# hvak/visual-underwater-slam

Hardware: AMD Instinct MI355X
Metric: ORB detect+match frames/sec (higher is better)
Workload: dtype u8

## Files before the change

### visual-underwater-slam_amd/_lib.py

```python
import ctypes
import os
from ctypes import c_int, c_void_p, c_char_p, c_double

_HERE = os.path.dirname(os.path.abspath(__file__))
LIB_PATH = os.environ.get("VUS_HIP_LIB") or os.path.join(_HERE, "csrc", "libvus_hip.so")

_P = c_void_p

SIGNATURES = {
    "vus_fast_score": [_P, c_int, c_int, c_int, c_int, c_int, _P, _P],
    "vus_blur7": [_P, c_int, c_int, c_int, c_int, _P, _P],
    "vus_fast_detect": [_P, c_int, c_int, c_int, c_int, c_int, c_int, _P, _P, c_int, _P, _P],
    "vus_fast_threshold_estimate": [_P, c_int, c_int, c_int, c_int, c_int, c_int, c_int, c_int, _P, _P, _P],
    "vus_fast_detect_adaptive": [_P, c_int, c_int, c_int, c_int, _P, c_int, _P, _P, c_int, _P, _P],
    "vus_fast_detect_retry": [_P, c_int, c_int, c_int, c_int, c_int, _P, c_int, c_int, _P, c_int, _P, _P, _P, _P],
    "vus_select_topk": [_P, _P, c_int, c_int, c_int, _P, _P, _P],
    "vus_orient_rbrief": [_P, _P, c_int, c_int, c_int, c_int, _P, _P, c_int, _P, _P, _P],
    "vus_orient_order": [_P, _P, c_int, c_int, c_int, c_int, _P, _P],
    "vus_orient_rbrief_ordered": [_P, _P, c_int, c_int, c_int, c_int, _P, _P, c_int, _P, _P, _P, _P],
    "vus_hamming_match": [_P, _P, _P, c_int, c_int, c_int, _P, _P, c_int, c_int, c_int, c_int, c_int, _P, _P, _P],
    "vus_triangulate": [_P, c_int, _P, _P, _P, _P],
    "vus_select_grid": [_P, _P, c_int, c_int, c_int, c_int, c_int, c_int, c_int, c_int, _P, _P, _P],
    "vus_cross_check": [_P, _P, c_int, c_int, _P, _P],
    "vus_resize_bilinear": [_P, c_int, c_int, c_int, c_int, _P, c_int, c_int, c_int, _P],
    "vus_pyramid_append": [_P, _P, _P, _P, c_int, c_int, c_int, c_int, c_int, c_int, c_int, c_int, _P, _P, _P, _P, _P, _P,
                           _P],
    "vus_track_ids": [_P, _P, _P, _P, c_int, c_int, c_int, c_int, _P, _P, _P, _P],
    "vus_stereo_initial_residuals": [_P, _P, _P, _P, _P, _P, c_int, _P, _P],
    "vus_emit_stereo_factors": [_P, _P, _P, _P, c_int, c_int, c_int, ctypes.c_longlong, _P, _P, _P, _P, _P, _P, _P, _P],
    "vus_ba_linearize": [_P, _P, _P, _P, _P, _P, _P, _P, _P, _P, _P],
    "vus_ba_schur": [_P, _P, c_double, _P, _P, _P, _P, _P, _P, _P, _P, c_int, _P, _P, _P],
    "vus_ba_tiles_count": [_P, _P, _P],
    "vus_ba_tiles_fill": [_P, c_int, _P, c_int, _P, _P, _P, _P, ctypes.c_longlong, _P],
    "vus_ba_add_diag": [_P, c_int, c_int, c_double, _P],
    "vus_ba_band_solve": [_P, c_int, c_int, _P, _P, _P, _P],
    "vus_ba_backsub": [_P, _P, _P, _P, _P, _P, _P],
    "vus_ba_eval_step": [_P, _P, _P, _P, _P, _P, _P, _P, _P, _P],
    "vus_ba_error": [_P, _P, _P, _P, _P, _P],
    "vus_ba_band_solve_multi": [_P, c_int, c_int, _P, c_int, _P, _P],
    "vus_ba_band_solve_split": [_P, c_int, c_int, _P, _P, _P, _P, _P],
    "vus_ba_band_solve_multi_split": [_P, c_int, c_int, _P, c_int, _P, _P, _P],
    "vus_ba_linearize_robust": [_P, _P, _P, _P, _P, _P, _P, _P, _P, _P, _P, _P],
    "vus_ba_eval_step_robust": [_P, _P, _P, _P, _P, _P, _P, _P, _P, _P, _P],
    "vus_ba_error_robust": [_P, _P, _P, _P, _P, _P, _P],
    "vus_ba_stereo_weights": [_P, _P, _P, _P, _P, _P],
    "vus_imu_preintegrate": [_P, _P, c_int, _P, _P, _P, _P],
    "vus_keys_to_indices": [_P, c_int, _P, _P, _P, _P, ctypes.c_longlong, _P],
    "vus_lookup_keys": [_P, c_int, _P, c_int, _P, _P, _P],
    "vus_ba_pack_observations": [_P, _P, _P, c_int, c_int, c_int, _P, _P, _P, _P, _P, _P, _P, _P, _P, _P, _P, ctypes.c_longlong, _P],
    "vus_exclusive_scan_i32": [_P, c_int, _P, _P, _P],
    "vus_nav_linearize": [_P, c_int, _P, _P, _P, _P, _P, _P, _P, _P, _P, _P, _P],
    "vus_nav_assemble": [c_int, c_int, c_double, _P, _P, _P, _P, _P, _P, _P],
    "vus_nav_border_solve": [c_int, _P, _P, _P, _P, c_double, _P, _P, _P],
    "vus_nav_eval_step": [_P, c_int, _P, _P, _P, _P, _P, _P, _P, _P, _P, _P, _P],
    "vus_nav_error": [_P, c_int, _P, _P, _P, _P, _P, _P],
    "vus_navb_linearize": [_P, c_int, _P, _P, _P, _P, _P, _P, _P, _P],
    "vus_navb_assemble": [c_int, c_int, c_double, _P, _P, _P, _P, _P],
    "vus_navb_eval_step": [_P, c_int, _P, _P, _P, _P, _P, _P, _P, _P, _P, _P],
    "vus_navb_error": [_P, c_int, _P, _P, _P, _P, _P, _P],
    "vus_ba_band_selinv": [_P, c_int, c_int, _P, _P, ctypes.c_longlong, _P],
    "vus_ba_point_check": [_P, c_int, _P, _P],
    "vus_ba_point_covariance": [_P, _P, _P, _P, _P, c_int, _P, _P],
    "vus_nav_border_covariance": [c_int, c_int, _P, _P, _P, _P, _P, _P, _P, _P],
    "vus_between_check": [_P, c_int, _P],
    "vus_between_linearize": [_P, _P, _P, _P, _P, _P],
    "vus_between_assemble": [_P, _P, c_int, _P, _P, _P],
    "vus_between_eval_step": [_P, _P, _P, _P, _P, _P, _P],
    "vus_between_error": [_P, _P, _P, _P, _P],
    "vus_ba_set_tuning": [c_int, c_int],
}

TUNE_BAND_MODE, TUNE_CB_MAX_WG, TUNE_LAST_BAND_MODE, TUNE_WIN_FAULT = 0, 1, 2, 3
STATUS_WAIT_EXPIRED, STATUS_WINDOW_EXPIRED = -1, -3


class VusError(RuntimeError):
    """A libvus_hip.so entry point returned a negative code (gtsam raises RuntimeError likewise)."""


_lib = None


def load():
    global _lib
    if _lib is not None:
        return _lib
    import torch
    if not os.path.exists(LIB_PATH):
        raise ImportError(
            f"{LIB_PATH} is missing: build it with `python -c 'import __graft_entry__ as g; g.build()'` "
            "or `make -C visual-underwater-slam_amd/csrc`. There is no CPU fallback.")
    lib = ctypes.CDLL(LIB_PATH)
    lib.vus_abi_version.restype = c_int
    lib.vus_last_error.restype = c_char_p
    lib.vus_build_target.restype = c_char_p
    for name, argtypes in SIGNATURES.items():
        fn = getattr(lib, name)
        fn.argtypes = argtypes
        fn.restype = c_int
    lib.vus_ba_work_doubles.argtypes = [_P]
    lib.vus_ba_work_doubles.restype = ctypes.c_longlong
    lib.vus_ba_band_solve_work_doubles.argtypes = [c_int, c_int, c_int]
    lib.vus_ba_band_solve_work_doubles.restype = ctypes.c_longlong
    lib.vus_pack_work_bytes.argtypes = [c_int]
    lib.vus_pack_work_bytes.restype = ctypes.c_longlong
    lib.vus_ba_tiles_work_bytes.argtypes = [c_int]
    lib.vus_ba_tiles_work_bytes.restype = ctypes.c_longlong
    lib.vus_ba_get_tuning.argtypes = [c_int]
    lib.vus_ba_get_tuning.restype = c_int
    lib.vus_nav_work_doubles.argtypes = [_P]
    lib.vus_nav_work_doubles.restype = ctypes.c_longlong
    lib.vus_navb_work_doubles.argtypes = [_P]
    lib.vus_navb_work_doubles.restype = ctypes.c_longlong
    lib.vus_between_work_doubles.argtypes = [_P]
    lib.vus_between_work_doubles.restype = ctypes.c_longlong
    lib.vus_ba_band_selinv_work_doubles.argtypes = [c_int, c_int]
    lib.vus_ba_band_selinv_work_doubles.restype = ctypes.c_longlong
    _lib = lib
    return lib


def call(name, *args):
    lib = load()
    rc = getattr(lib, name)(*args)
    if rc != 0:
        raise VusError(f"{name} failed ({rc}): {_explain_missing_code_object(lib.vus_last_error().decode())}")


def ptr(t):
    return None if t is None else t.data_ptr()


def current_stream_ptr():
    import torch
    return torch.cuda.current_stream().cuda_stream


def target_mismatch(built: str, device_arch: str):
    b, d = built.split(":"), device_arch.split(":")
    if b[0] != d[0]:
        return (f"libvus_hip.so was built for {built} but the device is {device_arch}: this library targets MI355X "
                f"(gfx950) only")
    for feat in b[1:]:
        if feat not in d[1:]:
            return (f"libvus_hip.so was built for target ID {built} but the device runs {device_arch}: no code object "
                    f"matches (every launch would fail with 'no kernel image is available'). Rebuild with "
                    f"`make -C visual-underwater-slam_amd/csrc clean all OFFLOAD=--offload-arch={b[0]}`")
    return None


def _explain_missing_code_object(text: str) -> str:
    if "no kernel image" not in text and "invalid device function" not in text:
        return text
    try:
        import torch
        arch = getattr(torch.cuda.get_device_properties(torch.cuda.current_device()), "gcnArchName", "")
        why = target_mismatch(load().vus_build_target().decode(), arch) if arch else None
    except Exception:
        why = None
    return f"{text} -- {why}" if why else text


def check_target():
    import torch
    arch = getattr(torch.cuda.get_device_properties(torch.cuda.current_device()), "gcnArchName", "")
    why = target_mismatch(load().vus_build_target().decode(), arch) if arch else None
    if why:
        raise RuntimeError(why)


def require_gpu():
    import torch
    if not torch.cuda.is_available():
        raise RuntimeError("visual_underwater_slam_amd needs an MI355X (HIP device); no GPU is visible "
                           "and there is deliberately no CPU fallback.")
```

### visual-underwater-slam_amd/csrc/frontend.hip

```cpp
#include "vus_common.h"
#define VUS_TABLE_QUAL __device__ constexpr
#include "../../include/vus_orb_tables.h"

namespace {

#ifndef VUS_TW
#define VUS_TW 128
#endif
#ifndef VUS_TH
#define VUS_TH 24
#endif
constexpr int TW = VUS_TW;
constexpr int TH = VUS_TH;
#ifndef VUS_AB_TILE
static_assert(TW == VUS_FAST_TILE_W && TH == VUS_FAST_TILE_H, "the sampling pattern of vus_fast_threshold_estimate is part of the ABI");
#endif
#ifndef VUS_FAST_WPE
#define VUS_FAST_WPE 1
#endif
#ifndef VUS_NT
#define VUS_NT 256
#endif
constexpr int NTHREADS = VUS_NT;
constexpr int IMG_ROWS = TH + 8;
constexpr int IMG_DW = (TW + 16) / 4;
constexpr int SC_ROWS = TH + 2;
constexpr int SC_DW = (TW + 8) / 4;
constexpr int H_ROWS = TH + 6;
constexpr int H_DW = TW / 2;
constexpr int STRIPS = TW / 4;

__device__ __forceinline__ int clampi(int v, int lo, int hi) { return v < lo ? lo : (v > hi ? hi : v); }
__device__ __forceinline__ int min3i(int a, int b, int c) { return min(min(a, b), c); }
__device__ __forceinline__ int max3i(int a, int b, int c) { return max(max(a, b), c); }
__device__ __forceinline__ int byte_of(uint32_t w, int i) { return (int)((w >> (8 * i)) & 0xFFu); }

template <int E>
__device__ __forceinline__ int fast_score_strip(const uint32_t (&r)[7][3]) {
  constexpr int DX[16] = {0, 1, 2, 3, 3, 3, 2, 1, 0, -1, -2, -3, -3, -3, -2, -1};
  constexpr int DY[16] = {-3, -3, -2, -1, 0, 1, 2, 3, 3, 3, 2, 1, 0, -1, -2, -3};
  const int p = byte_of(r[3][1], E);
  int d[16];
#pragma unroll
  for (int k = 0; k < 16; ++k) {
    const int pos = 4 + E + DX[k];
    d[k] = byte_of(r[3 + DY[k]][pos >> 2], pos & 3) - p;
  }
  int mn3[16], mx3[16];
#pragma unroll
  for (int k = 0; k < 16; ++k) {
    mn3[k] = min3i(d[k], d[(k + 1) & 15], d[(k + 2) & 15]);
    mx3[k] = max3i(d[k], d[(k + 1) & 15], d[(k + 2) & 15]);
  }
  int best_bright = -(1 << 20), best_dark = 1 << 20;
#pragma unroll
  for (int k = 0; k < 16; ++k) {
    best_bright = max(best_bright, min3i(mn3[k], mn3[(k + 3) & 15], mn3[(k + 6) & 15]));
    best_dark = min(best_dark, max3i(mx3[k], mx3[(k + 3) & 15], mx3[(k + 6) & 15]));
  }
  return max(best_bright, -best_dark) - 1;
}

__device__ __forceinline__ int fast_score_bytes(const uint8_t* c, int rb) {
  constexpr int DX[16] = {0, 1, 2, 3, 3, 3, 2, 1, 0, -1, -2, -3, -3, -3, -2, -1};
  constexpr int DY[16] = {-3, -3, -2, -1, 0, 1, 2, 3, 3, 3, 2, 1, 0, -1, -2, -3};
  const int p = c[0];
  int d[16];
#pragma unroll
  for (int k = 0; k < 16; ++k) d[k] = (int)c[DY[k] * rb + DX[k]] - p;
  int mn3[16], mx3[16];
#pragma unroll
  for (int k = 0; k < 16; ++k) {
    mn3[k] = min3i(d[k], d[(k + 1) & 15], d[(k + 2) & 15]);
    mx3[k] = max3i(d[k], d[(k + 1) & 15], d[(k + 2) & 15]);
  }
  int best_bright = -(1 << 20), best_dark = 1 << 20;
#pragma unroll
  for (int k = 0; k < 16; ++k) {
    best_bright = max(best_bright, min3i(mn3[k], mn3[(k + 3) & 15], mn3[(k + 6) & 15]));
    best_dark = min(best_dark, max3i(mx3[k], mx3[(k + 3) & 15], mx3[(k + 6) & 15]));
  }
  return max(best_bright, -best_dark) - 1;
}

typedef short short2_t __attribute__((ext_vector_type(2)));
__device__ __forceinline__ int fast_score_pk(const uint32_t (&r)[7][3]) {
  constexpr int DX[16] = {0, 1, 2, 3, 3, 3, 2, 1, 0, -1, -2, -3, -3, -3, -2, -1};
  constexpr int DY[16] = {-3, -3, -2, -1, 0, 1, 2, 3, 3, 3, 2, 1, 0, -1, -2, -3};
  const int p = byte_of(r[3][1], 0);
  uint32_t nr[7][2];
#pragma unroll
  for (int k = 0; k < 7; ++k) {
    nr[k][0] = ~r[k][0];
    nr[k][1] = ~r[k][1];
  }
  short2_t v[16];
#pragma unroll
  for (int k = 0; k < 16; ++k) {
    const int pos = 4 + DX[k], row = 3 + DY[k], dw = pos >> 2, by = pos & 3;
    const uint32_t sel = (uint32_t)by | (0x0cu << 8) | ((uint32_t)(4 + by) << 16) | (0x0cu << 24);
    v[k] = __builtin_bit_cast(short2_t, __builtin_amdgcn_perm(nr[row][dw], r[row][dw], sel));
  }
  short2_t w2[16], w4[16], w8[16];
#pragma unroll
  for (int k = 0; k < 16; ++k) w2[k] = __builtin_elementwise_min(v[k], v[(k + 1) & 15]);
#pragma unroll
  for (int k = 0; k < 16; ++k) w4[k] = __builtin_elementwise_min(w2[k], w2[(k + 2) & 15]);
#pragma unroll
  for (int k = 0; k < 16; ++k) w8[k] = __builtin_elementwise_min(w4[k], w4[(k + 4) & 15]);
  short2_t best = __builtin_elementwise_min(w8[0], v[8]);
#pragma unroll
  for (int k = 1; k < 16; ++k) best = __builtin_elementwise_max(best, __builtin_elementwise_min(w8[k], v[(k + 8) & 15]));
  return max((int)best.x - p, (int)best.y - (255 - p)) - 1;
}

#ifndef VUS_FAST_PK
#define VUS_FAST_PK 0
#endif

template <int E>
__device__ __forceinline__ bool nms_keep(const uint32_t (&c)[3][3]) {
  const int s = byte_of(c[1][1], E);
  int m = 0;
#pragma unroll
  for (int dy = 0; dy < 3; ++dy)
#pragma unroll
    for (int dx = -1; dx <= 1; ++dx) {
      if (dy == 1 && dx == 0) continue;
      const int pos = 4 + E + dx;
      m = max(m, byte_of(c[dy][pos >> 2], pos & 3));
    }
  return s > m;
}

#ifndef VUS_FAST_STRIP
#define VUS_FAST_STRIP 1
#endif
#ifndef VUS_BLUR_MFMA
#define VUS_BLUR_MFMA 1
#endif
#ifndef VUS_FAST_LATE_BLUR
#define VUS_FAST_LATE_BLUR 1
#endif
constexpr int VUS_CAND_REGIONS = 8;
#ifndef VUS_FAST_SCORE_BYTES
#define VUS_FAST_SCORE_BYTES 1
#endif
#ifndef VUS_FAST_MM_BYTES
#define VUS_FAST_MM_BYTES 1
#endif
#ifndef VUS_FAST_DIAG
#define VUS_FAST_DIAG 1
#endif
struct BlurMfmaTable {
  uint64_t h[64];
  uint64_t v[2][64];
};
constexpr BlurMfmaTable make_blur_mfma_table() {
  constexpr int BW[7] = {18, 33, 49, 56, 49, 33, 18};
  BlurMfmaTable t{};
  for (int l = 0; l < 64; ++l) {
    const int g = l >> 4, m = l & 15;
    for (int sl = 0; sl < 8; ++sl) {
      const int d = 8 * g + sl - m - 5;
      if (d >= 0 && d <= 6) t.h[l] |= (uint64_t)BW[d] << (8 * sl);
      const int hrow = sl < 4 ? 4 * g + sl : 16 + 4 * g + (sl - 4);
      for (int nb = 0; nb < 2; ++nb) {
        const int dv = hrow - (16 * nb + m + 1);
        if (dv >= 0 && dv <= 6) t.v[nb][l] |= (uint64_t)BW[dv] << (8 * sl);
      }
    }
  }
  return t;
}
__device__ __attribute__((aligned(16))) const BlurMfmaTable g_blur_mfma_table = make_blur_mfma_table();
typedef int v4i32_t __attribute__((ext_vector_type(4)));

__device__ __forceinline__ void blur_tile_mfma(const uint32_t* s_img, uint8_t* __restrict__ blur_out, int n, int H, int W,
                                               int x0, int y0, int tid, int j_first, int j_step) {
  static_assert(IMG_ROWS == 32 && TW % 16 == 0 && (IMG_DW * 4) % 8 == 0, "blur_tile_mfma: K = the 32 staged rows");
  const int l = tid & 63, g = l >> 4, m = l & 15;
  const long bh = (long)g_blur_mfma_table.h[l];
  const long bv[2] = {(long)g_blur_mfma_table.v[0][l], (long)g_blur_mfma_table.v[1][l]};
  const uint8_t* img8 = reinterpret_cast<const uint8_t*>(s_img);
  constexpr unsigned long long SIGN = 0x8080808080808080ull;
#ifndef VUS_BLUR_UNROLL
#define VUS_BLUR_UNROLL 1
#endif
#pragma unroll VUS_BLUR_UNROLL
  for (int j = j_first; j < TW / 16; j += j_step) {
    v4i32_t ch[2];
#pragma unroll
    for (int mb = 0; mb < 2; ++mb) {
      const unsigned long long a =
          *reinterpret_cast<const unsigned long long*>(img8 + (16 * mb + m) * (IMG_DW * 4) + 16 * j + 8 * g) ^ SIGN;
      const v4i32_t c0 = {32768, 32768, 32768, 32768};
      ch[mb] = __builtin_amdgcn_mfma_i32_16x16x32_i8((long)a, bh, c0, 0, 0, 0);
    }
    uint32_t lo[2], hi[2];
#pragma unroll
    for (int mb = 0; mb < 2; ++mb) {
      const uint32_t t0 = __builtin_amdgcn_perm((uint32_t)ch[mb][1], (uint32_t)ch[mb][0], 0x05010400u);
      const uint32_t t1 = __builtin_amdgcn_perm((uint32_t)ch[mb][3], (uint32_t)ch[mb][2], 0x05010400u);
      lo[mb] = __builtin_amdgcn_perm(t1, t0, 0x05040100u);
      hi[mb] = __builtin_amdgcn_perm(t1, t0, 0x07060302u);
    }
    const long a_lo = (long)((((unsigned long long)lo[1] << 32) | lo[0]) ^ SIGN);
    const long a_hi = (long)((((unsigned long long)hi[1] << 32) | hi[0]) ^ SIGN);
#pragma unroll
    for (int nb = 0; nb < 2; ++nb) {
      const v4i32_t ci = {32768, 32768, 32768, 32768};
      const v4i32_t cl = {65536, 65536, 65536, 65536};
      const v4i32_t chi = __builtin_amdgcn_mfma_i32_16x16x32_i8(a_hi, bv[nb], ci, 0, 0, 0);
      const v4i32_t clo = __builtin_amdgcn_mfma_i32_16x16x32_i8(a_lo, bv[nb], cl, 0, 0, 0);
      uint32_t q[4];
#pragma unroll
      for (int r = 0; r < 4; ++r) q[r] = ((uint32_t)chi[r] << 8) + (uint32_t)clo[r];
      const uint32_t v = __builtin_amdgcn_perm(q[1], q[0], 0x0c0c0602u) | __builtin_amdgcn_perm(q[3], q[2], 0x06020c0cu);
      const int ly = 16 * nb + m, gy = y0 + ly, gx = x0 + 16 * j + 4 * g;
#ifdef VUS_BLUR_EXP_NOSTORE
      if (v != 0x12345678u) continue;
#endif
      if (ly < TH && gy < H) {
        uint8_t* o = blur_out + ((size_t)n * H + gy) * W + gx;
        if (gx + 3 < W) {
          __builtin_memcpy(o, &v, 4);
        } else {
#pragma unroll
          for (int e = 0; e < 4; ++e)
            if (gx + e < W) o[e] = (uint8_t)(v >> (8 * e));
        }
      }
    }
  }
}

#ifdef VUS_FAST_DEBUG_COUNT
__device__ unsigned long long g_fast_dbg[4];
extern "C" int vus_debug_fast_counters(unsigned long long* out, int reset) {
  if (hipMemcpyFromSymbol(out, HIP_SYMBOL(g_fast_dbg), sizeof(g_fast_dbg)) != hipSuccess) return -1;
  if (reset) { unsigned long long z[4] = {0, 0, 0, 0}; if (hipMemcpyToSymbol(HIP_SYMBOL(g_fast_dbg), z, sizeof(z)) != hipSuccess) return -1; }
  return 0;
}
#endif
template <bool WRITE_SCORE, bool DETECT, bool BLUR, bool HIST = false, bool REGIONS = false>
__device__ __forceinline__ void fast_tile_body(
    const uint8_t* __restrict__ img, int H, int W, int pitch, int thr, int border,
    uint8_t* __restrict__ score_out, uint8_t* __restrict__ blur_out,
    uint32_t* __restrict__ cand_keys, int cand_cap, int* __restrict__ cand_count, int* __restrict__ hist,
    int n, int tile, int tiles_x) {
  __shared__ __attribute__((aligned(8))) uint32_t s_img[IMG_ROWS * IMG_DW];
  __shared__ uint32_t s_score[(WRITE_SCORE || DETECT) ? SC_ROWS * SC_DW : 1];
  constexpr bool STRIP = VUS_FAST_STRIP && (WRITE_SCORE || DETECT);
  constexpr bool MFMA_BLUR = VUS_BLUR_MFMA && BLUR && IMG_ROWS == 32;
  constexpr int AUX_DW = STRIP ? (IMG_ROWS * IMG_DW + SC_ROWS * SC_DW + 1) / 2 : 2;
  __shared__ uint32_t s_h[(BLUR && !MFMA_BLUR && H_ROWS * H_DW > AUX_DW) ? H_ROWS * H_DW : AUX_DW];
  __shared__ uint16_t s_work[(WRITE_SCORE || DETECT) ? SC_ROWS * SC_DW * 4 : 2];
#if VUS_FAST_STRIP
  uint16_t* const s_mm = reinterpret_cast<uint16_t*>(s_h);
  uint16_t* const s_strip = s_mm + IMG_ROWS * IMG_DW;
  __shared__ int s_nstrip;
#endif
  __shared__ int s_cnt, s_base, s_nwork;
  constexpr bool LATE_BLUR = MFMA_BLUR && DETECT && !HIST && STRIP && VUS_FAST_LATE_BLUR;
  static_assert(IMG_ROWS * IMG_DW >= TW * TH / 4, "candidate list must fit in the image tile");
  static_assert(!LATE_BLUR || AUX_DW >= TW * TH / 4, "candidate list must fit in the strip tables' buffer");
  uint32_t* const s_keys = LATE_BLUR ? s_h : s_img;

  const int tid = threadIdx.x;
  const int x0 = (tile % tiles_x) * TW, y0 = (tile / tiles_x) * TH;
  const uint8_t* im = img + (size_t)n * H * pitch;

  {
    constexpr int RPP = NTHREADS / IMG_DW;
    const int col = tid % IMG_DW, r0 = tid / IMG_DW;
    const int gx = x0 - 8 + 4 * col;
    const bool fast = gx >= 0 && gx + 3 < W;
    const bool inside = x0 >= 8 && x0 + TW + 8 <= W && y0 >= 4 && y0 + TH + 4 <= H;
    if (r0 < RPP) {
      constexpr int NP = (IMG_ROWS + RPP - 1) / RPP;
      constexpr int LASTP = IMG_ROWS - (NP - 1) * RPP;
      uint32_t v[NP];
      if (inside) {
        const uint32_t off0 = (uint32_t)((y0 - 4 + r0) * pitch + gx);
        const uint32_t step = (uint32_t)(RPP * pitch);
#pragma unroll
        for (int k = 0; k < NP - 1; ++k) __builtin_memcpy(&v[k], im + (off0 + (uint32_t)k * step), 4);
        v[NP - 1] = 0u;
        if (r0 < LASTP) __builtin_memcpy(&v[NP - 1], im + (off0 + (uint32_t)(NP - 1) * step), 4);
      } else {
        const uint8_t* rp[NP];
#pragma unroll
        for (int k = 0; k < NP; ++k) rp[k] = im + (size_t)clampi(y0 - 4 + min(r0 + RPP * k, IMG_ROWS - 1), 0, H - 1) * pitch;
        if (fast) {
#pragma unroll
          for (int k = 0; k < NP; ++k) __builtin_memcpy(&v[k], rp[k] + gx, 4);
        } else {
          const int c0 = clampi(gx, 0, W - 1), c1 = clampi(gx + 1, 0, W - 1), c2 = clampi(gx + 2, 0, W - 1),
                    c3 = clampi(gx + 3, 0, W - 1);
          uint8_t q[NP][4];
#pragma unroll
          for (int k = 0; k < NP; ++k) { q[k][0] = rp[k][c0]; q[k][1] = rp[k][c1]; q[k][2] = rp[k][c2]; q[k][3] = rp[k][c3]; }
#pragma unroll
          for (int k = 0; k < NP; ++k)
            v[k] = (uint32_t)q[k][0] | ((uint32_t)q[k][1] << 8) | ((uint32_t)q[k][2] << 16) | ((uint32_t)q[k][3] << 24);
        }
      }
#pragma unroll
      for (int k = 0; k < NP; ++k) {
        const int row = r0 + RPP * k;
        if (row < IMG_ROWS) {
          s_img[row * IMG_DW + col] = v[k];
#if VUS_FAST_STRIP
          if (WRITE_SCORE || DETECT) {
            const int b0 = byte_of(v[k], 0), b1 = byte_of(v[k], 1), b2 = byte_of(v[k], 2), b3 = byte_of(v[k], 3);
            s_mm[row * IMG_DW + col] = (uint16_t)(min(min(b0, b1), min(b2, b3)) | (max(max(b0, b1), max(b2, b3)) << 8));
          }
#endif
        }
      }
    }
  }
  if (tid == 0) {
    s_cnt = 0; s_nwork = 0;
#if VUS_FAST_STRIP
    s_nstrip = 0;
#endif
  }
  __syncthreads();
#ifdef VUS_FAST_EXIT_AFTER
#define VUS_FAST_EXIT(N) do { if (VUS_FAST_EXIT_AFTER == (N)) return; } while (0)
#else
#define VUS_FAST_EXIT(N)
#endif
  VUS_FAST_EXIT(1);

  if (WRITE_SCORE || DETECT) {
#if VUS_FAST_STRIP
    constexpr int S_RPP = NTHREADS / SC_DW;
    constexpr int NIT = (SC_ROWS + S_RPP - 1) / S_RPP;
    const int sr0 = tid / SC_DW, ss = tid - sr0 * SC_DW;
    const int gx = x0 - 4 + 4 * ss;
    const bool col_ok = sr0 < S_RPP && gx + 3 >= 3 && gx < W - 3;
    const int ci0 = (sr0 + 3) * IMG_DW + ss;
    unsigned long long bal[NIT];
    bool pass[NIT];
#pragma unroll
    for (int it = 0; it < NIT; ++it) {
      const int sr = sr0 + it * S_RPP;
      pass[it] = false;
      if (sr0 < S_RPP && sr < SC_ROWS) {
        const int gy = y0 - 1 + sr;
        if (col_ok && gy >= 3 && gy < H - 3) {
          const int ci = ci0 + it * S_RPP * IMG_DW;
#if VUS_FAST_MM_BYTES
          const uint8_t* mm8 = reinterpret_cast<const uint8_t*>(s_mm) + 2 * ci;
          const int ma_lo = mm8[0], ma_hi = mm8[1], pmin = mm8[2], pmax = mm8[3], mc_lo = mm8[4], mc_hi = mm8[5];
          const int mn_lo = mm8[2 - 6 * IMG_DW], mn_hi = mm8[3 - 6 * IMG_DW], ms_lo = mm8[2 + 6 * IMG_DW], ms_hi = mm8[3 + 6 * IMG_DW];
          const uint32_t b = s_img[ci + 1];
          const int b0 = byte_of(b, 0), b3 = byte_of(b, 3);
          const int hi = min(max(mn_hi, ms_hi), max3i(ma_hi, mc_hi, max(b0, b3)));
          const int lo = max(min(mn_lo, ms_lo), min3i(ma_lo, mc_lo, min(b0, b3)));
          pass[it] = hi > pmin + thr || lo < pmax - thr;
#else
          const int ma = s_mm[ci], mb = s_mm[ci + 1], mc = s_mm[ci + 2];
          const int mn = s_mm[ci + 1 - 3 * IMG_DW], ms = s_mm[ci + 1 + 3 * IMG_DW];
          const uint32_t b = s_img[ci + 1];
          const int b0 = byte_of(b, 0), b3 = byte_of(b, 3);
          const int pmin = mb & 0xFF, pmax = mb >> 8;
          const int hi = min(max(mn >> 8, ms >> 8), max3i(ma >> 8, mc >> 8, max(b0, b3)));
          const int lo = max(min(mn & 0xFF, ms & 0xFF), min3i(ma & 0xFF, mc & 0xFF, min(b0, b3)));
          pass[it] = hi > pmin + thr || lo < pmax - thr;
#endif
        }
        s_score[sr * SC_DW + ss] = 0u;
      }
      bal[it] = __ballot(pass[it]);
    }
    int total = 0;
#pragma unroll
    for (int it = 0; it < NIT; ++it) total += __popcll(bal[it]);
    if (total > 0) {
      int base = 0;
      if ((tid & 63) == 0) base = atomicAdd(&s_nstrip, total);
      base = __builtin_amdgcn_readfirstlane(base);
#pragma unroll
      for (int it = 0; it < NIT; ++it) {
        if (pass[it])
          s_strip[base + __builtin_amdgcn_mbcnt_hi((uint32_t)(bal[it] >> 32), __builtin_amdgcn_mbcnt_lo((uint32_t)bal[it], 0))] =
              (uint16_t)((sr0 + it * S_RPP) * SC_DW + ss);
        base += __popcll(bal[it]);
      }
    }
    __syncthreads();
    VUS_FAST_EXIT(2);
    const int nstrip = s_nstrip;
#ifdef VUS_FAST_DEBUG_COUNT
    if (tid == 0 && BLUR) { atomicAdd(&g_fast_dbg[0], 1ull); atomicAdd(&g_fast_dbg[1], (unsigned long long)nstrip); }
#endif
    for (int j0 = 0; j0 < nstrip; j0 += NTHREADS) {
      const int j = j0 + tid;
      int mask = 0, idx = 0;
      if (j < nstrip) {
        idx = s_strip[j];
        const int sr = idx / SC_DW, ss = idx - sr * SC_DW;
        const int gx = x0 - 4 + 4 * ss;
        {
#else
    for (int idx0 = 0; idx0 < SC_ROWS * SC_DW; idx0 += NTHREADS) {
      const int idx = idx0 + tid;
      int mask = 0;
      if (idx < SC_ROWS * SC_DW) {
        const int sr = idx / SC_DW, ss = idx - sr * SC_DW;
        const int gy = y0 - 1 + sr, gx = x0 - 4 + 4 * ss;
        if (gy >= 3 && gy < H - 3 && gx + 3 >= 3 && gx < W - 3) {
#endif
          const uint32_t* cp = &s_img[(sr + 3) * IMG_DW + ss];
          const uint32_t a = cp[0], b = cp[1], c = cp[2];
          const uint32_t nn = s_img[sr * IMG_DW + ss + 1], so = s_img[(sr + 6) * IMG_DW + ss + 1];
          const uint32_t wv = __builtin_amdgcn_alignbyte(b, a, 1);
          const uint32_t ev = __builtin_amdgcn_alignbyte(c, b, 3);
#if VUS_FAST_DIAG
          const uint32_t* up = &s_img[(sr + 1) * IMG_DW + ss];
          const uint32_t* dn = &s_img[(sr + 5) * IMG_DW + ss];
          const uint32_t nev = __builtin_amdgcn_alignbyte(up[2], up[1], 2), nwv = __builtin_amdgcn_alignbyte(up[1], up[0], 2);
          const uint32_t sev = __builtin_amdgcn_alignbyte(dn[2], dn[1], 2), swv = __builtin_amdgcn_alignbyte(dn[1], dn[0], 2);
#endif
#pragma unroll
          for (int e = 0; e < 4; ++e) {
            const int p = byte_of(b, e);
            const int n_ = byte_of(nn, e), s_ = byte_of(so, e), w_ = byte_of(wv, e), e_ = byte_of(ev, e);
            int hi = min(max(n_, s_), max(e_, w_)), lo = max(min(n_, s_), min(e_, w_));
#if VUS_FAST_DIAG
            const int ne = byte_of(nev, e), sw = byte_of(swv, e), se = byte_of(sev, e), nw = byte_of(nwv, e);
            hi = min3i(hi, max(ne, sw), max(se, nw));
            lo = max3i(lo, min(ne, sw), min(se, nw));
#endif
            mask |= (hi > p + thr || lo < p - thr) ? (1 << e) : 0;
          }
          if (gx < 3 || gx + 3 >= W - 3) {
#pragma unroll
            for (int e = 0; e < 4; ++e)
              if (gx + e < 3 || gx + e >= W - 3) mask &= ~(1 << e);
          }
        }
#if !VUS_FAST_STRIP
        s_score[idx] = 0u;
#endif
      }
      const int cnt = __popc(mask);
      int incl = cnt;
      incl += __builtin_amdgcn_update_dpp(0, incl, 0x111, 0xf, 0xf, true);
      incl += __builtin_amdgcn_update_dpp(0, incl, 0x112, 0xf, 0xf, true);
      incl += __builtin_amdgcn_update_dpp(0, incl, 0x114, 0xf, 0xe, true);
      incl += __builtin_amdgcn_update_dpp(0, incl, 0x118, 0xf, 0xc, true);
      incl += __builtin_amdgcn_update_dpp(0, incl, 0x142, 0xa, 0xf, true);
      incl += __builtin_amdgcn_update_dpp(0, incl, 0x143, 0xc, 0xf, true);
      const int total = __builtin_amdgcn_readlane(incl, 63);
      int base = 0;
      if ((tid & 63) == 0 && total > 0) base = atomicAdd(&s_nwork, total);
      base = __builtin_amdgcn_readfirstlane(base);
      int pos = base + incl - cnt;
#pragma unroll
      for (int e = 0; e < 4; ++e)
        if (mask & (1 << e)) s_work[pos++] = (uint16_t)(idx * 4 + e);
    }
  }
  auto blur_rows = [&]() {
    constexpr uint32_t W0123 = 18u | (33u << 8) | (49u << 16) | (56u << 24);
    constexpr uint32_t W456 = 49u | (33u << 8) | (18u << 16);
    for (int idx = tid; idx < H_ROWS * STRIPS; idx += NTHREADS) {
      const int hr = idx / STRIPS, hs = idx - hr * STRIPS;
      const uint32_t* rp = &s_img[(hr + 1) * IMG_DW + hs + 1];
      const uint32_t a = rp[0], b = rp[1], c = rp[2];
      const uint32_t o0 = __builtin_amdgcn_udot4(__builtin_amdgcn_alignbyte(b, a, 1), W0123, 0u, false) +
                          __builtin_amdgcn_udot4(__builtin_amdgcn_alignbyte(c, b, 1), W456, 0u, false);
      const uint32_t o1 = __builtin_amdgcn_udot4(__builtin_amdgcn_alignbyte(b, a, 2), W0123, 0u, false) +
                          __builtin_amdgcn_udot4(__builtin_amdgcn_alignbyte(c, b, 2), W456, 0u, false);
      const uint32_t o2 = __builtin_amdgcn_udot4(__builtin_amdgcn_alignbyte(b, a, 3), W0123, 0u, false) +
                          __builtin_amdgcn_udot4(__builtin_amdgcn_alignbyte(c, b, 3), W456, 0u, false);
      const uint32_t o3 = __builtin_amdgcn_udot4(b, W0123, 0u, false) + __builtin_amdgcn_udot4(c, W456, 0u, false);
      uint2 out = make_uint2(o0 | (o1 << 16), o2 | (o3 << 16));
      *reinterpret_cast<uint2*>(&s_h[hr * H_DW + 2 * hs]) = out;
    }
  };
#ifdef VUS_FAST_DEBUG_COUNT
  __syncthreads();
  if (tid == 0 && BLUR && (WRITE_SCORE || DETECT)) atomicAdd(&g_fast_dbg[2], (unsigned long long)s_nwork);
#endif
  VUS_FAST_EXIT(3);
  if (BLUR && !MFMA_BLUR && !STRIP) blur_rows();
  if (MFMA_BLUR && !LATE_BLUR) blur_tile_mfma(s_img, blur_out, n, H, W, x0, y0, tid, tid >> 6, NTHREADS / 64);
  __syncthreads();
  VUS_FAST_EXIT(4);

  if (BLUR && !MFMA_BLUR && STRIP) blur_rows();
  if (WRITE_SCORE || DETECT) {
    const int nwork = s_nwork;
    uint8_t* score8 = reinterpret_cast<uint8_t*>(s_score);
    for (int j = tid; j < nwork; j += NTHREADS) {
      const int ent = s_work[j];
      const int idx = ent >> 2, e = ent & 3;
      const int sr = idx / SC_DW, ss = idx - sr * SC_DW;
#if VUS_FAST_SCORE_BYTES
      const int sc = fast_score_bytes(reinterpret_cast<const uint8_t*>(s_img) + (sr + 3) * (4 * IMG_DW) + 4 * (ss + 1) + e, 4 * IMG_DW);
#else
      uint32_t r[7][3];
#pragma unroll
      for (int k = 0; k < 7; ++k) {
        const uint32_t* rp = &s_img[(sr + k) * IMG_DW + ss];
        const uint32_t a = rp[0], b = rp[1], c = rp[2];
        r[k][0] = __builtin_amdgcn_alignbyte(b, a, e);
        r[k][1] = __builtin_amdgcn_alignbyte(c, b, e);
        r[k][2] = c >> (8 * e);
      }
#if VUS_FAST_PK
      const int sc = fast_score_pk(r);
#else
      const int sc = fast_score_strip<0>(r);
#endif
#endif
      if (sc >= thr) score8[ent] = (uint8_t)sc;
    }
    __syncthreads();
  }
  VUS_FAST_EXIT(5);

  if (WRITE_SCORE) {
    for (int idx = tid; idx < TH * STRIPS; idx += NTHREADS) {
      const int ly = idx / STRIPS, ls = idx - ly * STRIPS;
      const int gy = y0 + ly, gx = x0 + 4 * ls;
      const uint32_t v = s_score[(ly + 1) * SC_DW + ls + 1];
      if (gy < H) {
        uint8_t* o = score_out + ((size_t)n * H + gy) * W + gx;
#pragma unroll
        for (int e = 0; e < 4; ++e)
          if (gx + e < W) o[e] = (uint8_t)(v >> (8 * e));
      }
    }
  }
  if (BLUR && !MFMA_BLUR) {
    constexpr int BW[7] = {18, 33, 49, 56, 49, 33, 18};
    for (int idx = tid; idx < TH * STRIPS; idx += NTHREADS) {
      const int ly = idx / STRIPS, ls = idx - ly * STRIPS;
      const int gy = y0 + ly, gx = x0 + 4 * ls;
      uint32_t a0 = 0, a1 = 0, a2 = 0, a3 = 0;
#pragma unroll
      for (int k = 0; k < 7; ++k) {
        const uint2 h = *reinterpret_cast<const uint2*>(&s_h[(ly + k) * H_DW + 2 * ls]);
        a0 += (uint32_t)BW[k] * (h.x & 0xFFFFu);
        a1 += (uint32_t)BW[k] * (h.x >> 16);
        a2 += (uint32_t)BW[k] * (h.y & 0xFFFFu);
        a3 += (uint32_t)BW[k] * (h.y >> 16);
      }
      const uint32_t v = ((a0 + 32768u) >> 16) | (((a1 + 32768u) >> 16) << 8) | (((a2 + 32768u) >> 16) << 16) |
                         (((a3 + 32768u) >> 16) << 24);
      if (gy < H) {
        uint8_t* o = blur_out + ((size_t)n * H + gy) * W + gx;
        if (gx + 3 < W) {
          __builtin_memcpy(o, &v, 4);
        } else {
#pragma unroll
          for (int e = 0; e < 4; ++e)
            if (gx + e < W) o[e] = (uint8_t)(v >> (8 * e));
        }
      }
    }
  }
  if (DETECT) {
    const int nwork = s_nwork;
    const uint8_t* score8 = reinterpret_cast<const uint8_t*>(s_score);
    for (int j = tid; j < nwork; j += NTHREADS) {
      const int ent = s_work[j];
      const int s = score8[ent];
      if (s == 0) continue;
      const int sr = ent / (4 * SC_DW), sx = ent - sr * (4 * SC_DW);
      const int ly = sr - 1, lx = sx - 4;
      if (ly < 0 || ly >= TH || lx < 0 || lx >= TW) continue;
      const int gy = y0 + ly, gx = x0 + lx;
      if (gy < border || gy >= H - border || gx < border || gx >= W - border) continue;
      const uint8_t* c = score8 + ent;
      constexpr int RB = 4 * SC_DW;
      const int m = max(max3i(c[-RB - 1], c[-RB], c[-RB + 1]), max(max(c[-1], c[1]), max3i(c[RB - 1], c[RB], c[RB + 1])));
      if (s > m) {
        if (HIST) {
          atomicAdd(&hist[256 * n + s], 1);
        } else {
          const int p = atomicAdd(&s_cnt, 1);
          s_keys[p] = ((uint32_t)(255 - s) << VUS_KEY_POS_BITS) | (uint32_t)(gy * W + gx);
        }
      }
    }
    if (!HIST) {
      __syncthreads();
      const int cnt = s_cnt;
      const int rcap = cand_cap / VUS_CAND_REGIONS;
      uint32_t* const list = cand_keys + (size_t)n * cand_cap + (REGIONS ? (size_t)(tile & (VUS_CAND_REGIONS - 1)) * rcap : 0);
      int* const counter = REGIONS ? reinterpret_cast<int*>(list) : &cand_count[n];
      if (LATE_BLUR) {
        if (tid == NTHREADS - 64 && cnt > 0) s_base = atomicAdd(counter, cnt);
        if (tid < NTHREADS - 64) blur_tile_mfma(s_img, blur_out, n, H, W, x0, y0, tid, tid >> 6, NTHREADS / 64 - 1);
      } else {
        if (tid == 0 && cnt > 0) s_base = atomicAdd(counter, cnt);
      }
      __syncthreads();
      if (cnt > 0) {
        const int base = s_base + (REGIONS ? 1 : 0), lim = REGIONS ? rcap : cand_cap;
        for (int i = tid; i < cnt; i += NTHREADS)
          if (base + i < lim) list[base + i] = s_keys[i];
      }
    }
  }
}

template <bool WRITE_SCORE, bool DETECT, bool BLUR, bool REGIONS = false>
__global__ __launch_bounds__(NTHREADS, VUS_FAST_WPE) void fast_tile_kernel(
    const uint8_t* __restrict__ img, int H, int W, int pitch, int thr, const int* __restrict__ thr_img, int border,
    uint8_t* __restrict__ score_out, uint8_t* __restrict__ blur_out,
    uint32_t* __restrict__ cand_keys, int cand_cap, int* __restrict__ cand_count, int n_img, int tiles_x,
    int tiles_per_img) {
  const int xcd = blockIdx.x & 7, slot = blockIdx.x >> 3;
  const int n = (slot / tiles_per_img) * 8 + xcd;
  if (n >= n_img) return;
  const int tile = slot - (slot / tiles_per_img) * tiles_per_img;
  fast_tile_body<WRITE_SCORE, DETECT, BLUR, false, REGIONS>(img, H, W, pitch, thr_img ? thr_img[n] : thr, border, score_out, blur_out,
                                                            cand_keys, cand_cap, cand_count, nullptr, n, tile, tiles_x);
}

__global__ void cand_region_zero_kernel(uint32_t* __restrict__ cand_keys, int cand_cap, int n_img) {
  const int t = blockIdx.x * blockDim.x + threadIdx.x;
  if (t < n_img * VUS_CAND_REGIONS)
    cand_keys[(size_t)(t / VUS_CAND_REGIONS) * cand_cap + (size_t)(t % VUS_CAND_REGIONS) * (cand_cap / VUS_CAND_REGIONS)] = 0u;
}

__global__ __launch_bounds__(256) void cand_region_merge_kernel(uint32_t* __restrict__ cand_keys, int cand_cap, int* __restrict__ cand_count) {
  __shared__ int s_c[VUS_CAND_REGIONS];
  const int n = blockIdx.x, tid = threadIdx.x;
  const int rcap = cand_cap / VUS_CAND_REGIONS;
  uint32_t* row = cand_keys + (size_t)n * cand_cap;
  if (tid < VUS_CAND_REGIONS) s_c[tid] = (int)row[(size_t)tid * rcap];
  __syncthreads();
  int off = 0;
  long long all = 0;
  bool over = false;
  for (int r = 0; r < VUS_CAND_REGIONS; ++r) {
    const int c = s_c[r], m = min(c, rcap - 1);
    all += c;
    over |= c > rcap - 1;
    const uint32_t* src = row + (size_t)r * rcap + 1;
    for (int i0 = 0; i0 < m; i0 += 256) {
      const int i = i0 + tid;
      const uint32_t v = i < m ? src[i] : 0u;
      __syncthreads();
      if (i < m) row[off + i] = v;
      __syncthreads();
    }
    off += m;
  }
  if (over)
    for (int i = off + tid; i < cand_cap; i += 256) row[i] = VUS_KEY_INVALID;
  if (tid == 0) cand_count[n] = over ? (int)max(all, (long long)cand_cap + 1) : off;
}

__global__ __launch_bounds__(NTHREADS, VUS_FAST_WPE) void fast_sample_kernel(const uint8_t* __restrict__ img, int H, int W, int pitch,
                                                               int thr, int border, int* __restrict__ hist, int n_img,
                                                               int tiles_x, int tiles_per_img, int stride, int n_sampled) {
  const int xcd = blockIdx.x & 7, slot = blockIdx.x >> 3;
  const int n = (slot / n_sampled) * 8 + xcd;
  if (n >= n_img) return;
  const int tile = (slot - (slot / n_sampled) * n_sampled) * stride + stride / 2;
  if (tile >= tiles_per_img) return;
  fast_tile_body<false, true, false, true>(img, H, W, pitch, thr, border, nullptr, nullptr, nullptr, 0, nullptr, hist, n, tile, tiles_x);
}

__global__ __launch_bounds__(256) void fast_pick_threshold_kernel(const int* __restrict__ hist, int n_img, int thr, int floor, int max_kp,
                                                                  long long n_tiles, long long n_sampled, int num, int den,
                                                                  int* __restrict__ thr_img) {
  const int n = blockIdx.x * 4 + (threadIdx.x >> 6), lane = threadIdx.x & 63;
  if (n >= n_img) return;
  const int4 h = reinterpret_cast<const int4*>(hist + 256 * (size_t)n)[lane];
  const int hv[4] = {h.x, h.y, h.z, lane == 63 ? 0 : h.w};
  int above = hv[0] + hv[1] + hv[2] + hv[3];
  int incl = above;
#pragma unroll
  for (int d = 1; d < 64; d <<= 1) {
    const int o = __shfl_down(incl, d);
    if (lane + d < 64) incl += o;
  }
  above = incl - above;
  const long long need = (long long)max_kp * n_sampled * num;
  long long run = above;
  int best = -1;
#pragma unroll
  for (int q = 3; q >= 0; --q) {
    run += hv[q];
    const int t = 4 * lane + q;
    if (best < 0 && t > floor && t <= 254 && run * n_tiles * den >= need) best = t;
  }
#pragma unroll
  for (int d = 32; d >= 1; d >>= 1) best = max(best, __shfl_xor(best, d));
  if (lane == 0) thr_img[n] = best > floor ? best : thr;
}

__global__ __launch_bounds__(1024) void fast_retry_list_kernel(const int* __restrict__ thr_img, int thr, int max_kp, int n_img,
                                                               int* __restrict__ cand_count, int* __restrict__ retry_list,
                                                               int* __restrict__ retry_count) {
  __shared__ int s_n;
  if (threadIdx.x == 0) s_n = 0;
  __syncthreads();
  for (int n = threadIdx.x; n < n_img; n += 1024)
    if (thr_img[n] > thr && cand_count[n] < max_kp) {
      retry_list[atomicAdd(&s_n, 1)] = n;
      cand_count[n] = 0;
    }
  __syncthreads();
  if (threadIdx.x == 0) retry_count[0] = s_n;
}

__global__ __launch_bounds__(NTHREADS, VUS_FAST_WPE) void fast_retry_kernel(const uint8_t* __restrict__ img, int H, int W, int pitch, int thr,
                                                              int border, uint32_t* __restrict__ cand_keys, int cand_cap,
                                                              int* __restrict__ cand_count, const int* __restrict__ retry_list,
                                                              const int* __restrict__ retry_count, int tiles_x, int tiles_per_img) {
  const long long items = (long long)retry_count[0] * tiles_per_img;
  for (long long it = blockIdx.x; it < items; it += gridDim.x) {
    const int n = retry_list[it / tiles_per_img], tile = (int)(it % tiles_per_img);
    fast_tile_body<false, true, false>(img, H, W, pitch, thr, border, nullptr, nullptr, cand_keys, cand_cap, cand_count, nullptr, n,
                                       tile, tiles_x);
    __syncthreads();
  }
}

constexpr int SEL_THREADS = 1024;

__global__ __launch_bounds__(SEL_THREADS) void select_topk_kernel(
    const uint32_t* __restrict__ cand_keys, const int* __restrict__ cand_count, int cand_cap,
    int max_kp, int sort_n, uint32_t* __restrict__ kp_keys, int* __restrict__ kp_count) {
  extern __shared__ uint32_t s_sort[];
  __shared__ int s_hist[256];
  __shared__ int s_scan[256];
  __shared__ int s_wtot[4];
  __shared__ uint32_t s_prefix;
  __shared__ int s_k, s_out;
  const int tid = threadIdx.x;
  const int n = blockIdx.x;
  const uint32_t* keys = cand_keys + (size_t)n * cand_cap;
  const int cnt = min(cand_count[n], cand_cap);
  const int K = min(cnt, max_kp);

  uint32_t T = 0xFFFFFFFFu;
  if (cnt > max_kp) {
    if (tid == 0) { s_prefix = 0; s_k = max_kp; }
    uint32_t mask = 0;
    for (int shift = 24; shift >= 0; shift -= 8) {
      for (int i = tid; i < 256; i += SEL_THREADS) s_hist[i] = 0;
      __syncthreads();
      const uint32_t prefix = s_prefix;
      for (int i = tid; i < cnt; i += SEL_THREADS) {
        uint32_t k = keys[i];
        if ((k & mask) == prefix) atomicAdd(&s_hist[(k >> shift) & 255], 1);
      }
      __syncthreads();
      const int kk = s_k;
      __syncthreads();
      if (tid < 256) {
        const int h = s_hist[tid];
        int incl = h;
        incl += __builtin_amdgcn_update_dpp(0, incl, 0x111, 0xf, 0xf, true);
        incl += __builtin_amdgcn_update_dpp(0, incl, 0x112, 0xf, 0xf, true);
        incl += __builtin_amdgcn_update_dpp(0, incl, 0x114, 0xf, 0xe, true);
        incl += __builtin_amdgcn_update_dpp(0, incl, 0x118, 0xf, 0xc, true);
        incl += __builtin_amdgcn_update_dpp(0, incl, 0x142, 0xa, 0xf, true);
        incl += __builtin_amdgcn_update_dpp(0, incl, 0x143, 0xc, 0xf, true);
        if ((tid & 63) == 63) s_wtot[tid >> 6] = incl;
        s_scan[tid] = incl;
      }
      __syncthreads();
      if (tid < 256) {
        int base = 0;
        for (int w = 0; w < (tid >> 6); ++w) base += s_wtot[w];
        const int incl = s_scan[tid] + base, excl = incl - s_hist[tid];
        if (excl < kk && kk <= incl) {
          s_prefix = prefix | ((uint32_t)tid << shift);
          s_k = kk - excl;
        }
      }
      mask |= 0xFFu << shift;
      __syncthreads();
    }
    T = s_prefix;
  }
  for (int i = tid; i < sort_n; i += SEL_THREADS) s_sort[i] = VUS_KEY_INVALID;
  if (tid == 0) s_out = 0;
  __syncthreads();
  for (int i = tid; i < cnt; i += SEL_THREADS) {
    uint32_t k = keys[i];
    if (k <= T) {
      int p = atomicAdd(&s_out, 1);
      if (p < sort_n) s_sort[p] = k;
    }
  }
  __syncthreads();
  for (int k = 2; k <= sort_n; k <<= 1) {
    for (int j = k >> 1; j > 0; j >>= 1) {
      for (int i = tid; i < sort_n; i += SEL_THREADS) {
        int l = i ^ j;
        if (l > i) {
          uint32_t a = s_sort[i], b = s_sort[l];
          bool up = (i & k) == 0;
          if ((a > b) == up) { s_sort[i] = b; s_sort[l] = a; }
        }
      }
      __syncthreads();
    }
  }
  for (int i = tid; i < max_kp; i += SEL_THREADS)
    kp_keys[(size_t)n * max_kp + i] = i < K ? s_sort[i] : VUS_KEY_INVALID;
  if (tid == 0) kp_count[n] = K;
}

constexpr int OR_R = 15;
constexpr int OR_ROWS = 2 * OR_R + 1;
#ifndef VUS_OR_VW
#define VUS_OR_VW 2
#endif
constexpr int OR_VW = VUS_OR_VW;
constexpr int OR_DW = OR_VW == 4 ? 12 : 10;
constexpr int BR_R = VUS_RBRIEF_REACH;
constexpr int BR_ROWS = 2 * BR_R + 1;
constexpr int BR_DW = OR_VW == 4 ? 12 : 10;
#ifndef VUS_OR_KPW
#define VUS_OR_KPW 8
#endif
constexpr int OR_KP_PER_WAVE = VUS_OR_KPW;

template <int VW> struct PatchVec;
template <> struct PatchVec<2> { typedef uint32_t type __attribute__((ext_vector_type(2), aligned(1))); };
template <> struct PatchVec<4> { typedef uint32_t type __attribute__((ext_vector_type(4), aligned(1))); };

template <int RADIUS, int DW, int VW, bool EXACT>
struct PatchRegs {
  static_assert(DW % VW == 0, "row width must be a multiple of the vector width");
  typedef typename PatchVec<VW>::type vec_t;
  static constexpr int ROWS = 2 * RADIUS + 1;
  static constexpr int HW = DW / VW;
  static constexpr int N = ROWS * HW;
  static constexpr int ITERS = (N + 63) / 64;
  vec_t v[ITERS];
  uint32_t off[ITERS];

  __device__ __forceinline__ void init(int pitch, int lane) {
#pragma unroll
    for (int u = 0; u < ITERS; ++u) {
      const int t = min(lane + 64 * u, N - 1);
      off[u] = (uint32_t)((t / HW) * pitch + 4 * VW * (t % HW));
    }
  }
  __device__ __forceinline__ void load(const uint8_t* __restrict__ src, int H, int W, int pitch, int y, int x,
                                       int lane) {
    const int xa = EXACT ? x - RADIUS : (x - RADIUS) & ~3;
    const bool inside = y - RADIUS >= 0 && y + RADIUS < H && xa >= 0 && xa + 4 * DW <= W;
    if (inside) {
      const uint8_t* base = src + (size_t)(y - RADIUS) * pitch + xa;
#pragma unroll
      for (int u = 0; u < ITERS; ++u) v[u] = *reinterpret_cast<const vec_t*>(base + (size_t)off[u]);
    } else {
#pragma unroll
      for (int u = 0; u < ITERS; ++u) {
        const int t = min(lane + 64 * u, N - 1);
        const int r = t / HW, c = t - r * HW;
        const uint8_t* rp = src + (size_t)clampi(y - RADIUS + r, 0, H - 1) * pitch;
        const int gx = xa + 4 * VW * c;
#pragma unroll
        for (int k = 0; k < VW; ++k)
          v[u][k] = (uint32_t)rp[clampi(gx + 4 * k, 0, W - 1)] | ((uint32_t)rp[clampi(gx + 4 * k + 1, 0, W - 1)] << 8) |
                    ((uint32_t)rp[clampi(gx + 4 * k + 2, 0, W - 1)] << 16) |
                    ((uint32_t)rp[clampi(gx + 4 * k + 3, 0, W - 1)] << 24);
      }
    }
  }
  __device__ __forceinline__ void store(uint32_t* __restrict__ dst, int lane) const {
#pragma unroll
    for (int u = 0; u < ITERS; ++u)
      if (lane + 64 * u < N) {
        uint32_t* d = dst + VW * (lane + 64 * u);
#pragma unroll
        for (int k = 0; k < VW; k += 2) *reinterpret_cast<uint2*>(d + k) = make_uint2(v[u][k], v[u][k + 1]);
      }
  }
};

__device__ __forceinline__ int fold32(int x, int y) {
  auto r = __builtin_amdgcn_permlane32_swap((uint32_t)x, (uint32_t)y, false, false);
  return (int)(r[0] + r[1]);
}
__device__ __forceinline__ int fold16(int x, int y) {
  auto r = __builtin_amdgcn_permlane16_swap((uint32_t)x, (uint32_t)y, false, false);
  return (int)(r[0] + r[1]);
}
template <int CTRL>
__device__ __forceinline__ int dpp_i32(int v) { return __builtin_amdgcn_update_dpp(0, v, CTRL, 0xf, 0xf, true); }
constexpr int DPP_ROW_ROR8 = 0x128, DPP_HALF_MIRROR = 0x141, DPP_QUAD_XOR1 = 0xB1, DPP_QUAD_XOR2 = 0x4E;
__device__ __forceinline__ int fold8(int x, int y, bool upper8) {
  const int keep = upper8 ? y : x, give = upper8 ? x : y;
  return keep + dpp_i32<DPP_ROW_ROR8>(give);
}
__device__ __forceinline__ int allsum8(int v) {
  v += dpp_i32<DPP_HALF_MIRROR>(v);
  v += dpp_i32<DPP_QUAD_XOR1>(v);
  v += dpp_i32<DPP_QUAD_XOR2>(v);
  return v;
}
template <int CTRL>
__device__ __forceinline__ long long dpp_max_i64(long long key) {
  const int lo = dpp_i32<CTRL>((int)(uint32_t)key), hi = dpp_i32<CTRL>((int)(key >> 32));
  const long long ok = (long long)(((unsigned long long)(uint32_t)hi << 32) | (uint32_t)lo);
  return ok > key ? ok : key;
}
__device__ __forceinline__ long long allmax8_i64(long long key) {
  key = dpp_max_i64<DPP_HALF_MIRROR>(key);
  key = dpp_max_i64<DPP_QUAD_XOR1>(key);
  key = dpp_max_i64<DPP_QUAD_XOR2>(key);
  return key;
}

__device__ __forceinline__ uint32_t writelane_u32(uint32_t reg, uint32_t value, int lane_sel) {
  asm("s_mov_b32 m0, %2\n\tv_writelane_b32 %0, %1, m0" : "+v"(reg) : "s"(value), "s"(lane_sel));
  return reg;
}


struct RotOffTable {
  uint32_t v[VUS_N_ANGLE_BINS * 64 * 4];
};
constexpr RotOffTable make_rot_off_table() {
  RotOffTable r{};
  for (int e = 0; e < VUS_N_ANGLE_BINS * 256; ++e) {
    const int bin = e / 256, test = e - 256 * bin, w = test >> 6, lane = test & 63;
    const int oa = VUS_RBRIEF_ROT[4 * e + 1] * (4 * BR_DW) + VUS_RBRIEF_ROT[4 * e];
    const int ob = VUS_RBRIEF_ROT[4 * e + 3] * (4 * BR_DW) + VUS_RBRIEF_ROT[4 * e + 2];
    r.v[(bin * 64 + lane) * 4 + w] = ((uint32_t)oa & 0xFFFFu) | ((uint32_t)ob << 16);
  }
  return r;
}
__device__ __attribute__((aligned(16))) const RotOffTable g_rot_off_table = make_rot_off_table();

#ifndef VUS_OR_WPE
#define VUS_OR_WPE 4
#endif
#ifndef VUS_OR_GRP
#define VUS_OR_GRP 4
#endif
constexpr int OR_GRP = VUS_OR_GRP;
static_assert(OR_VW == 2 && OR_KP_PER_WAVE == 8, "orient_rbrief_kernel is written for dwordx2 patch loads and 8 keypoints per wave");
constexpr int OR_NV = OR_ROWS * (OR_DW / OR_VW);
constexpr int OR_WT = 192;

struct DiscWeightTable {
  uint32_t v[4 * OR_WT * 4];
};
constexpr DiscWeightTable make_disc_weight_table() {
  constexpr int umax[16] = {15, 15, 15, 15, 14, 14, 14, 13, 13, 12, 11, 10, 9, 8, 6, 3};
  DiscWeightTable r{};
  for (int e = 0; e < 4 * OR_WT; ++e) {
    const int sh = e / OR_WT, t = e - sh * OR_WT;
    if (t >= OR_NV) continue;
    const int row = t / (OR_DW / 2), c = t - row * (OR_DW / 2);
    const int dy = row - OR_R, um = umax[dy < 0 ? -dy : dy];
    for (int d = 0; d < 2; ++d)
      for (int b = 0; b < 4; ++b) {
        const int dx = 4 * (2 * c + d) + b - sh - OR_R;
        if (dx >= -um && dx <= um) {
          r.v[4 * e + d] |= (uint32_t)(dx + OR_R) << (8 * b);
          r.v[4 * e + 2 + d] |= 1u << (8 * b);
        }
      }
  }
  return r;
}
__device__ __attribute__((aligned(16))) const DiscWeightTable g_disc_weight_table = make_disc_weight_table();

constexpr int OO_CELL = 64, OO_MAX_CELLS = 1024;
__global__ __launch_bounds__(256) void orient_order_kernel(const uint32_t* __restrict__ kp_keys, const int* __restrict__ kp_count,
                                                           int max_kp, int W, int cw, int n_cells, int* __restrict__ order) {
  __shared__ int s_cnt[OO_MAX_CELLS];
  __shared__ int s_wave[4];
  const int n = blockIdx.x, tid = threadIdx.x;
  const int cnt = min(kp_count[n], max_kp);
  const uint32_t* keys = kp_keys + (size_t)n * max_kp;
  int* ord = order + (size_t)n * max_kp;
  for (int r = tid; r < n_cells; r += 256) s_cnt[r] = 0;
  __syncthreads();
  for (int j = tid; j < cnt; j += 256) {
    const uint32_t pos = keys[j] & VUS_KEY_POS_MASK;
    const int y = (int)(pos / (uint32_t)W), x = (int)(pos - (uint32_t)y * (uint32_t)W);
    atomicAdd(&s_cnt[(y / OO_CELL) * cw + (x / OO_CELL)], 1);
  }
  __syncthreads();
  int c[4], sum = 0;
#pragma unroll
  for (int q = 0; q < 4; ++q) {
    c[q] = 4 * tid + q < n_cells ? s_cnt[4 * tid + q] : 0;
    sum += c[q];
  }
  int incl = sum;
#pragma unroll
  for (int d = 1; d < 64; d <<= 1) {
    const int o = __shfl_up(incl, d);
    if ((tid & 63) >= d) incl += o;
  }
  if ((tid & 63) == 63) s_wave[tid >> 6] = incl;
  __syncthreads();
  int base = incl - sum;
  for (int w = 0; w < (tid >> 6); ++w) base += s_wave[w];
#pragma unroll
  for (int q = 0; q < 4; ++q)
    if (4 * tid + q < n_cells) {
      s_cnt[4 * tid + q] = base;
      base += c[q];
    }
  __syncthreads();
  for (int j = tid; j < cnt; j += 256) {
    const uint32_t pos = keys[j] & VUS_KEY_POS_MASK;
    const int y = (int)(pos / (uint32_t)W), x = (int)(pos - (uint32_t)y * (uint32_t)W);
    ord[atomicAdd(&s_cnt[(y / OO_CELL) * cw + (x / OO_CELL)], 1)] = j;
  }
  for (int j = cnt + tid; j < max_kp; j += 256) ord[j] = j;
}

template <bool EXACT, bool ORDERED>
__global__ __launch_bounds__(256) __attribute__((amdgpu_waves_per_eu(VUS_OR_WPE, 8))) void orient_rbrief_kernel(
    const uint8_t* __restrict__ img, const uint8_t* __restrict__ blur, int H, int W, int pitch,
    const uint32_t* __restrict__ kp_keys, const int* __restrict__ kp_count, int max_kp, const int* __restrict__ order,
    uint64_t* __restrict__ desc_out, uint8_t* __restrict__ angle_out, int n_img, int chunks_per_img) {
  __shared__ uint4 s_w[4 * OR_WT];
  __shared__ __attribute__((aligned(8))) uint32_t s_blur[4][2][BR_ROWS * BR_DW];
  const int lane = threadIdx.x & 63;
  const int wave = __builtin_amdgcn_readfirstlane(threadIdx.x >> 6);
  const int xcd = blockIdx.x & 7, slot = blockIdx.x >> 3;
  const int n = (slot / chunks_per_img) * 8 + xcd;
  const int chunk = slot - (slot / chunks_per_img) * chunks_per_img;
  if (n >= n_img) return;
  {
    const uint4* wt = reinterpret_cast<const uint4*>(g_disc_weight_table.v);
#pragma unroll
    for (int i = 0; i < 4 * OR_WT / 256; ++i) s_w[threadIdx.x + 256 * i] = wt[threadIdx.x + 256 * i];
  }
  const uint8_t* im = img + (size_t)n * H * pitch;
  const uint8_t* bl = blur + (size_t)n * H * W;
  const int base_i = (chunk * 4 + wave) * OR_KP_PER_WAVE;
  const int n_live = clampi(min(kp_count[n], max_kp) - base_i, 0, OR_KP_PER_WAVE);
  int my_y = 0, my_x = 0;
  int my_idx = base_i + lane;
  if (ORDERED && lane < OR_KP_PER_WAVE && base_i + lane < max_kp) my_idx = order[(size_t)n * max_kp + base_i + lane];
  if (lane < n_live) {
    const uint32_t pos = kp_keys[(size_t)n * max_kp + my_idx] & VUS_KEY_POS_MASK;
    my_y = (int)(pos / (uint32_t)W);
    my_x = (int)(pos - (uint32_t)my_y * (uint32_t)W);
  }
  int bin_cos[4], bin_sin[4];
#pragma unroll
  for (int q = 0; q < 4; ++q) {
    const int bq = min(4 * (lane & 7) + q, VUS_N_ANGLE_BINS - 1);
    bin_cos[q] = VUS_ANGLE_COS[bq];
    bin_sin[q] = VUS_ANGLE_SIN[bq];
  }
  PatchRegs<OR_R, OR_DW, OR_VW, EXACT> pr[OR_GRP];
  PatchRegs<BR_R, BR_DW, OR_VW, EXACT> pb;
#pragma unroll
  for (int kk = 0; kk < OR_GRP; ++kk) pr[kk].init(pitch, lane);
  pb.init(W, lane);
  int mom_dy[3];
#pragma unroll
  for (int u = 0; u < 3; ++u) mom_dy[u] = min(lane + 64 * u, OR_NV - 1) / (OR_DW / 2) - OR_R;
  __syncthreads();
  if (n_live == 0) {
    if (lane < 4 * OR_KP_PER_WAVE && base_i + (lane >> 2) < max_kp) desc_out[((size_t)n * max_kp + base_i) * 4 + lane] = 0;
    if (lane < OR_KP_PER_WAVE && base_i + lane < max_kp) angle_out[(size_t)n * max_kp + base_i + lane] = 0;
    return;
  }

  int pa[8], pq[8];
#pragma unroll
  for (int g = 0; g < 8 / OR_GRP; ++g) {
#pragma unroll
    for (int kk = 0; kk < OR_GRP; ++kk) {
      const int k = OR_GRP * g + kk;
#ifndef VUS_OR_EXP_NORAW
      if (k < n_live)
        pr[kk].load(im, H, W, pitch, __builtin_amdgcn_readlane(my_y, k), __builtin_amdgcn_readlane(my_x, k), lane);
#else
      for (int u = 0; u < 3; ++u) pr[kk].v[u] = typename PatchVec<OR_VW>::type{(uint32_t)lane, (uint32_t)k};
#endif
    }
    if (g == 8 / OR_GRP - 1)
      pb.load(bl, H, W, W, __builtin_amdgcn_readlane(my_y, 0), __builtin_amdgcn_readlane(my_x, 0), lane);
#pragma unroll
    for (int kk = 0; kk < OR_GRP; ++kk) {
      const int k = OR_GRP * g + kk;
      pa[k] = 0;
      pq[k] = 0;
      if (k < n_live) {
        const int sh = EXACT ? 0 : (__builtin_amdgcn_readlane(my_x, k) - OR_R) & 3;
        const uint4* wt = s_w + sh * OR_WT + lane;
        uint32_t sx = 0;
        int si = 0, sy = 0;
#pragma unroll
        for (int u = 0; u < 3; ++u) {
          const uint4 w = wt[64 * u];
          sx = __builtin_amdgcn_udot4(pr[kk].v[u][0], w.x, sx, false);
          sx = __builtin_amdgcn_udot4(pr[kk].v[u][1], w.y, sx, false);
          uint32_t rs = __builtin_amdgcn_udot4(pr[kk].v[u][0], w.z, 0u, false);
          rs = __builtin_amdgcn_udot4(pr[kk].v[u][1], w.w, rs, false);
          si += (int)rs;
          sy += mom_dy[u] * (int)rs;
        }
        pa[k] = (int)sx - OR_R * si;
        pq[k] = sy;
      }
    }
  }
  int m10, m01;
  {
    const bool up8 = (lane & 8) != 0;
    int c[4], d[2];
#pragma unroll
    for (int j = 0; j < 4; ++j) c[j] = fold32(pa[j], pa[j + 4]);
#pragma unroll
    for (int j = 0; j < 2; ++j) d[j] = fold16(c[j], c[j + 2]);
    m10 = allsum8(fold8(d[0], d[1], up8));
#pragma unroll
    for (int j = 0; j < 4; ++j) c[j] = fold32(pq[j], pq[j + 4]);
#pragma unroll
    for (int j = 0; j < 2; ++j) d[j] = fold16(c[j], c[j + 2]);
    m01 = allsum8(fold8(d[0], d[1], up8));
  }
  int my_bin;
  {
    long long best = (long long)(-0x7FFFFFFFFFFFFFFFll - 1);
#pragma unroll
    for (int q = 0; q < 4; ++q) {
      const int bq = 4 * (lane & 7) + q;
      long long key = ((long long)m10 * bin_cos[q] + (long long)m01 * bin_sin[q]) * 32 + (31 - bq);
      if (bq >= VUS_N_ANGLE_BINS) key = (long long)(-0x7FFFFFFFFFFFFFFFll - 1);
      best = key > best ? key : best;
    }
    best = allmax8_i64(best);
    my_bin = 31 - (int)(best & 31);
  }
  {
    const int j_ang = ORDERED ? __shfl(my_idx, lane >> 3) : base_i + (lane >> 3);
    if ((lane & 7) == 0 && base_i + (lane >> 3) < max_kp) angle_out[(size_t)n * max_kp + j_ang] = (uint8_t)my_bin;
  }

  uint32_t wlo = 0, whi = 0;
  const uint4* rot = reinterpret_cast<const uint4*>(g_rot_off_table.v) + lane;
  uint4 to = rot[__builtin_amdgcn_readlane(my_bin, 0) * 64];
  for (int k = 0; k < n_live; ++k) {
    uint32_t* patch = s_blur[wave][k & 1];
    pb.store(patch, lane);
    const uint4 cto = to;
    const int cx = __builtin_amdgcn_readlane(my_x, k);
    if (k + 1 < n_live) {
#ifndef VUS_OR_EXP_NOBLUR
      pb.load(bl, H, W, W, __builtin_amdgcn_readlane(my_y, k + 1), __builtin_amdgcn_readlane(my_x, k + 1), lane);
#endif
      to = rot[__builtin_amdgcn_readlane(my_bin, 8 * (k + 1)) * 64];
    }
    __builtin_amdgcn_fence(__ATOMIC_ACQ_REL, "wavefront");
    const int sh_blur = EXACT ? 0 : (cx - BR_R) & 3;
    const uint8_t* c = reinterpret_cast<const uint8_t*>(patch) + BR_R * (4 * BR_DW) + BR_R + sh_blur;
    const uint32_t tw[4] = {cto.x, cto.y, cto.z, cto.w};
#pragma unroll
    for (int w = 0; w < 4; ++w) {
      const int a = c[(int16_t)(tw[w] & 0xFFFFu)];
      const int b = c[(int16_t)(tw[w] >> 16)];
      const uint64_t word = __ballot(a < b);
      wlo = writelane_u32(wlo, (uint32_t)word, 4 * k + w);
      whi = writelane_u32(whi, (uint32_t)(word >> 32), 4 * k + w);
    }
    __builtin_amdgcn_fence(__ATOMIC_ACQ_REL, "wavefront");
  }
  const int j_desc = ORDERED ? __shfl(my_idx, lane >> 2) : 0;
  if (lane < 4 * OR_KP_PER_WAVE && base_i + (lane >> 2) < max_kp)
    desc_out[ORDERED ? ((size_t)n * max_kp + j_desc) * 4 + (lane & 3) : ((size_t)n * max_kp + base_i) * 4 + lane] =
        ((uint64_t)whi << 32) | wlo;
}

#ifndef VUS_MT
#define VUS_MT 512
#endif
constexpr int MT = VUS_MT;

template <bool GATE>
__global__ __launch_bounds__(256) void hamming_match_kernel(
    const uint64_t* __restrict__ desc, const uint32_t* __restrict__ kp_keys,
    const int* __restrict__ kp_count, int max_kp, int W, const int* __restrict__ q_index,
    const int* __restrict__ t_index, int max_dy, int min_disp, int max_disp, int max_dist,
    int32_t* __restrict__ idx_out, int32_t* __restrict__ dist_out) {
  __shared__ uint64_t s_desc[MT * 4];
  __shared__ int s_xy[MT];
  const int tid = threadIdx.x;
  const int p = blockIdx.y;
  const int qi = q_index[p], ti = t_index[p];
  const int i = blockIdx.x * 256 + tid;
  const int nq = kp_count[qi], nt = kp_count[ti];
  const bool active = i < nq;
  uint64_t q0 = 0, q1 = 0, q2 = 0, q3 = 0;
  int yq = 0, xq = 0;
  if (active) {
    const uint64_t* dq = desc + ((size_t)qi * max_kp + i) * 4;
    q0 = dq[0]; q1 = dq[1]; q2 = dq[2]; q3 = dq[3];
    uint32_t pq = kp_keys[(size_t)qi * max_kp + i] & VUS_KEY_POS_MASK;
    yq = (int)(pq / (uint32_t)W);
    xq = (int)(pq - (uint32_t)yq * (uint32_t)W);
  }
  int best = 1 << 20, bidx = -1;
  const uint64_t* dt = desc + (size_t)ti * max_kp * 4;
  const uint32_t* kt = kp_keys + (size_t)ti * max_kp;
  for (int t0 = 0; t0 < nt; t0 += MT) {
    const int tn = min(MT, nt - t0);
    __syncthreads();
    for (int k = tid; k < tn * 4; k += 256) s_desc[k] = dt[(size_t)t0 * 4 + k];
    for (int k = tid; k < tn; k += 256) {
      uint32_t pt = kt[t0 + k] & VUS_KEY_POS_MASK;
      int yt = (int)(pt / (uint32_t)W);
      s_xy[k] = (yt << 16) | (int)(pt - (uint32_t)yt * (uint32_t)W);
    }
    __syncthreads();
    if (active) {
      for (int j = 0; j < tn; ++j) {
        int dist = __popcll(q0 ^ s_desc[4 * j]) + __popcll(q1 ^ s_desc[4 * j + 1]) +
                   __popcll(q2 ^ s_desc[4 * j + 2]) + __popcll(q3 ^ s_desc[4 * j + 3]);
        bool ok = true;
        if (GATE) {
          int xy = s_xy[j];
          int dy = yq - (int)((unsigned)xy >> 16), dx = xq - (xy & 0xFFFF);
          ok = dy <= max_dy && dy >= -max_dy && dx >= min_disp && dx <= max_disp;
        }
        if (ok && dist < best) { best = dist; bidx = t0 + j; }
      }
    }
  }
  if (i < max_kp) {
    if (bidx < 0) best = 512;
    else if (best > max_dist) bidx = -1;
    idx_out[(size_t)p * max_kp + i] = bidx;
    dist_out[(size_t)p * max_kp + i] = best;
  }
}

__global__ __launch_bounds__(256) void hamming_match_rows_kernel(
    const uint64_t* __restrict__ desc, const uint32_t* __restrict__ kp_keys,
    const int* __restrict__ kp_count, int max_kp, int W, int Hrows, const int* __restrict__ q_index,
    const int* __restrict__ t_index, int max_dy, int min_disp, int max_disp, int max_dist,
    int32_t* __restrict__ idx_out, int32_t* __restrict__ dist_out) {
  extern __shared__ int s_dyn[];
  int* s_start = s_dyn;
  int* s_cursor = s_dyn + (Hrows + 1);
  int* s_list = s_cursor + Hrows;
  int* s_xy = s_list + max_kp;
  __shared__ int s_wsum[4];
  const int tid = threadIdx.x;
  const int p = blockIdx.y;
  const int qi = q_index[p], ti = t_index[p];
  const int i = blockIdx.x * 256 + tid;
  const int nq = min(kp_count[qi], max_kp), nt = min(kp_count[ti], max_kp);
  const uint32_t* kt = kp_keys + (size_t)ti * max_kp;
  for (int r = tid; r <= Hrows; r += 256) s_start[r] = 0;
  __syncthreads();
  for (int j = tid; j < nt; j += 256) {
    const uint32_t pt = kt[j] & VUS_KEY_POS_MASK;
    const int yt = min((int)(pt / (uint32_t)W), Hrows - 1);
    s_xy[j] = (yt << 16) | (int)(pt - (uint32_t)(pt / (uint32_t)W) * (uint32_t)W);
    atomicAdd(&s_start[yt + 1], 1);
  }
  __syncthreads();
  {
    const int per = (Hrows + 255) / 256;
    const int b = 1 + tid * per, e = min(Hrows + 1, b + per);
    int sum = 0;
    for (int r = b; r < e; ++r) sum += s_start[r];
    int incl = sum;
#pragma unroll
    for (int o = 1; o < 64; o <<= 1) {
      int v = __shfl_up(incl, o);
      if ((tid & 63) >= o) incl += v;
    }
    if ((tid & 63) == 63) s_wsum[tid >> 6] = incl;
    __syncthreads();
    int base = incl - sum;
    for (int w = 0; w < (tid >> 6); ++w) base += s_wsum[w];
    for (int r = b; r < e; ++r) { base += s_start[r]; s_start[r] = base; }
  }
  __syncthreads();
  for (int r = tid; r < Hrows; r += 256) s_cursor[r] = s_start[r];
  __syncthreads();
  for (int j = tid; j < nt; j += 256) s_list[atomicAdd(&s_cursor[s_xy[j] >> 16], 1)] = j;
  __syncthreads();

  int best = 1 << 20, bidx = -1;
  if (i < nq) {
    const uint64_t* dq = desc + ((size_t)qi * max_kp + i) * 4;
    const uint64_t q0 = dq[0], q1 = dq[1], q2 = dq[2], q3 = dq[3];
    const uint32_t pq = kp_keys[(size_t)qi * max_kp + i] & VUS_KEY_POS_MASK;
    const int yq = (int)(pq / (uint32_t)W), xq = (int)(pq - (uint32_t)yq * (uint32_t)W);
    const int r0 = max(0, yq - max_dy), r1 = min(Hrows - 1, yq + max_dy);
    const uint64_t* dt = desc + (size_t)ti * max_kp * 4;
    if (r0 <= r1) {
      for (int c = s_start[r0]; c < s_start[r1 + 1]; ++c) {
        const int j = s_list[c];
        const int dx = xq - (s_xy[j] & 0xFFFF);
        if (dx < min_disp || dx > max_disp) continue;
        const uint64_t* d = dt + (size_t)j * 4;
        const int dist = __popcll(q0 ^ d[0]) + __popcll(q1 ^ d[1]) + __popcll(q2 ^ d[2]) + __popcll(q3 ^ d[3]);
        if (dist < best || (dist == best && j < bidx)) { best = dist; bidx = j; }
      }
    }
  }
  if (i < max_kp) {
    if (bidx < 0) best = 512;
    else if (best > max_dist) bidx = -1;
    idx_out[(size_t)p * max_kp + i] = bidx;
    dist_out[(size_t)p * max_kp + i] = best;
  }
}

constexpr int TRK_THREADS = 1024;
__global__ __launch_bounds__(TRK_THREADS) void track_ids_kernel(
    const int32_t* __restrict__ stereo_idx, const int32_t* __restrict__ track_idx,
    const uint32_t* __restrict__ kp_keys, const int* __restrict__ kp_count, int n_frames, int max_kp, int H, int W,
    long long* __restrict__ ids_out, double* __restrict__ feat_out, long long* __restrict__ n_ids_out) {
  extern __shared__ long long s_trk[];
  long long* s_cur = s_trk;
  long long* s_nxt = s_trk + max_kp;
  int* s_src = reinterpret_cast<int*>(s_trk + 2 * max_kp);
  __shared__ int s_part[TRK_THREADS];
  __shared__ long long s_next;
  const int tid = threadIdx.x;
  const int per = (max_kp + TRK_THREADS - 1) / TRK_THREADS;
  if (tid == 0) s_next = 0;
  int n_prev = 0;
  for (int f = 0; f < n_frames; ++f) {
    const int nl = min(kp_count[2 * f], max_kp), nr = min(kp_count[2 * f + 1], max_kp);
    for (int i = tid; i < max_kp; i += TRK_THREADS) { s_nxt[i] = -1; s_src[i] = 0x7FFFFFFF; }
    __syncthreads();
    if (f > 0)
      for (int ip = tid; ip < n_prev; ip += TRK_THREADS) {
        const int j = track_idx[(size_t)(f - 1) * max_kp + ip];
        if (j >= 0 && j < nl && s_cur[ip] >= 0) atomicMin(&s_src[j], ip);
      }
    __syncthreads();
    for (int j = tid; j < nl; j += TRK_THREADS)
      if (s_src[j] != 0x7FFFFFFF) s_nxt[j] = s_cur[s_src[j]];
    __syncthreads();
    int local = 0;
    for (int u = 0; u < per; ++u) {
      const int i = tid * per + u;
      if (i < nl) {
        const int j = stereo_idx[(size_t)f * max_kp + i];
        local += (j >= 0 && j < nr && s_nxt[i] < 0) ? 1 : 0;
      }
    }
    s_part[tid] = local;
    __syncthreads();
    for (int o = 1; o < TRK_THREADS; o <<= 1) {
      const int v = tid >= o ? s_part[tid - o] : 0;
      __syncthreads();
      s_part[tid] += v;
      __syncthreads();
    }
    long long id = s_next + s_part[tid] - local;
    const long long total = s_part[TRK_THREADS - 1];
    const uint32_t* kl = kp_keys + (size_t)(2 * f) * max_kp;
    const uint32_t* kr = kp_keys + (size_t)(2 * f + 1) * max_kp;
    for (int u = 0; u < per; ++u) {
      const int i = tid * per + u;
      if (i >= max_kp) break;
      long long out_id = -1;
      double ft[4] = {0.0, 0.0, 0.0, 0.0};
      if (i < nl) {
        const int j = stereo_idx[(size_t)f * max_kp + i];
        if (j >= 0 && j < nr) {
          if (s_nxt[i] < 0) s_nxt[i] = id++;
          out_id = s_nxt[i];
          const uint32_t pl = kl[i] & VUS_KEY_POS_MASK, pr = kr[j] & VUS_KEY_POS_MASK;
          ft[0] = 2.0 * (double)(pl % (uint32_t)W) / (double)W - 1.0;
          ft[1] = 2.0 * (double)(pl / (uint32_t)W) / (double)H - 1.0;
          ft[2] = 2.0 * (double)(pr % (uint32_t)W) / (double)W - 1.0;
          ft[3] = 2.0 * (double)(pr / (uint32_t)W) / (double)H - 1.0;
        }
      }
      ids_out[(size_t)f * max_kp + i] = out_id;
      double* o = feat_out + ((size_t)f * max_kp + i) * 4;
      o[0] = ft[0]; o[1] = ft[1]; o[2] = ft[2]; o[3] = ft[3];
    }
    __syncthreads();
    for (int i = tid; i < max_kp; i += TRK_THREADS) s_cur[i] = s_nxt[i];
    if (tid == 0) s_next += total;
    n_prev = nl;
    __syncthreads();
  }
  if (tid == 0) n_ids_out[0] = s_next;
}

__global__ void triangulate_kernel(const double* __restrict__ feat, int n, const double* __restrict__ cam,
                                   const double* __restrict__ Rt, double* __restrict__ out) {
  int i = blockIdx.x * blockDim.x + threadIdx.x;
  if (i >= n) return;
  const double fx = cam[0], fy = cam[1], cx = cam[2], cy = cam[3], baseline = cam[4];
  const double res_x = cam[5], res_y = cam[6];
  const double f = (fx + fy) / 2.0;
  double u0 = feat[4 * i + 0], v0 = feat[4 * i + 1], u1 = feat[4 * i + 2], v1 = feat[4 * i + 3];
  double uL = (u0 + 1) * 0.5 * res_x;
  double uR = (u1 + 1) * 0.5 * res_x;
  double v = ((v0 + v1) / 2.0 + 1) * 0.5 * res_y;
  double d = uR - uL;
  double Wd = d / baseline;
  double xc = (uL - cx) / Wd, yc = (v - cy) / Wd, zc = f / Wd;
#pragma unroll
  for (int r = 0; r < 3; ++r)
    out[6 * i + r] = ((Rt[3 * r + 0] * xc + Rt[3 * r + 1] * yc) + Rt[3 * r + 2] * zc) + Rt[9 + r];
  out[6 * i + 3] = uL;
  out[6 * i + 4] = uR;
  out[6 * i + 5] = v;
}

__device__ __forceinline__ void triangulate_one(const double* __restrict__ ft, const double* __restrict__ cam,
                                                const double* __restrict__ Rt, double* out) {
  const double fx = cam[0], fy = cam[1], cx = cam[2], cy = cam[3], baseline = cam[4];
  const double res_x = cam[5], res_y = cam[6];
  const double f = (fx + fy) / 2.0;
  const double uL = (ft[0] + 1) * 0.5 * res_x;
  const double uR = (ft[2] + 1) * 0.5 * res_x;
  const double v = ((ft[1] + ft[3]) / 2.0 + 1) * 0.5 * res_y;
  const double d = uR - uL;
  const double Wd = d / baseline;
  const double xc = (uL - cx) / Wd, yc = (v - cy) / Wd, zc = f / Wd;
#pragma unroll
  for (int r = 0; r < 3; ++r) out[r] = ((Rt[3 * r + 0] * xc + Rt[3 * r + 1] * yc) + Rt[3 * r + 2] * zc) + Rt[9 + r];
  out[3] = uL;
  out[4] = uR;
  out[5] = v;
}

constexpr int EMIT_THREADS = 256;

__global__ __launch_bounds__(EMIT_THREADS) void emit_count_kernel(const long long* __restrict__ ids, int max_kp,
                                                                  int first_frame, long long n_ids,
                                                                  int* __restrict__ frame_count,
                                                                  unsigned long long* __restrict__ lm_first) {
  __shared__ int s_n;
  const int f = blockIdx.x;
  if (threadIdx.x == 0) s_n = 0;
  __syncthreads();
  int local = 0;
  if (f >= first_frame)
    for (int i = threadIdx.x; i < max_kp; i += EMIT_THREADS) {
      const long long id = ids[(size_t)f * max_kp + i];
      if (id >= 0 && id < n_ids) {
        ++local;
        atomicMin(&lm_first[id], (unsigned long long)f * (unsigned long long)max_kp + (unsigned long long)i);
      }
    }
  atomicAdd(&s_n, local);
  __syncthreads();
  if (threadIdx.x == 0) frame_count[f] = s_n;
}

__global__ __launch_bounds__(1024) void emit_scan_kernel(int* __restrict__ frame_base, int n_frames, int* __restrict__ count) {
  __shared__ int s_part[1024];
  const int tid = threadIdx.x;
  const int per = (n_frames + 1023) / 1024;
  int local = 0;
  for (int u = 0; u < per; ++u) {
    const int f = tid * per + u;
    if (f < n_frames) local += frame_base[f];
  }
  s_part[tid] = local;
  __syncthreads();
  for (int o = 1; o < 1024; o <<= 1) {
    const int v = tid >= o ? s_part[tid - o] : 0;
    __syncthreads();
    s_part[tid] += v;
    __syncthreads();
  }
  int run = s_part[tid] - local;
  for (int u = 0; u < per; ++u) {
    const int f = tid * per + u;
    if (f < n_frames) {
      const int c = frame_base[f];
      frame_base[f] = run;
      run += c;
    }
  }
  if (tid == 1023) {
    frame_base[n_frames] = s_part[1023];
    count[0] = s_part[1023];
  }
}

__global__ __launch_bounds__(EMIT_THREADS) void emit_write_kernel(const long long* __restrict__ ids,
                                                                  const double* __restrict__ feat,
                                                                  const double* __restrict__ Rt,
                                                                  const double* __restrict__ cam, int max_kp,
                                                                  int first_frame, long long n_ids,
                                                                  const int* __restrict__ frame_base,
                                                                  int* __restrict__ obs_frame,
                                                                  long long* __restrict__ obs_id,
                                                                  double* __restrict__ obs_meas,
                                                                  long long* __restrict__ lm_first,
                                                                  double* __restrict__ lm_point) {
  __shared__ int s_part[EMIT_THREADS];
  const int f = blockIdx.x, tid = threadIdx.x;
  if (f < first_frame) return;
  const int per = (max_kp + EMIT_THREADS - 1) / EMIT_THREADS;
  int local = 0;
  for (int u = 0; u < per; ++u) {
    const int i = tid * per + u;
    if (i < max_kp) {
      const long long id = ids[(size_t)f * max_kp + i];
      local += (id >= 0 && id < n_ids) ? 1 : 0;
    }
  }
  s_part[tid] = local;
  __syncthreads();
  for (int o = 1; o < EMIT_THREADS; o <<= 1) {
    const int v = tid >= o ? s_part[tid - o] : 0;
    __syncthreads();
    s_part[tid] += v;
    __syncthreads();
  }
  int pos = frame_base[f] + s_part[tid] - local;
  for (int u = 0; u < per; ++u) {
    const int i = tid * per + u;
    if (i >= max_kp) break;
    const long long id = ids[(size_t)f * max_kp + i];
    if (id < 0 || id >= n_ids) continue;
    double tri[6];
    triangulate_one(feat + ((size_t)f * max_kp + i) * 4, cam, Rt + 12 * (size_t)f, tri);
    obs_frame[pos] = f;
    obs_id[pos] = id;
    obs_meas[3 * (size_t)pos] = tri[3];
    obs_meas[3 * (size_t)pos + 1] = tri[4];
    obs_meas[3 * (size_t)pos + 2] = tri[5];
    if (lm_first[id] == (long long)f * max_kp + i) {
      lm_point[3 * (size_t)id] = tri[0];
      lm_point[3 * (size_t)id + 1] = tri[1];
      lm_point[3 * (size_t)id + 2] = tri[2];
    }
    ++pos;
  }
}

__global__ void stereo_initial_residuals_kernel(const double* __restrict__ Rt, const double* __restrict__ K,
                                                const double* __restrict__ lm_point, const int* __restrict__ obs_frame,
                                                const long long* __restrict__ obs_id, const double* __restrict__ obs_meas,
                                                int n, double* __restrict__ resid) {
  const int a = blockIdx.x * blockDim.x + threadIdx.x;
  if (a >= n) return;
  const double* T = Rt + 12 * (size_t)obs_frame[a];
  const double* p = lm_point + 3 * (size_t)obs_id[a];
  const double fx = K[0], fy = K[1], cx = K[3], cy = K[4], b = K[5];
  const double d0 = p[0] - T[9], d1 = p[1] - T[10], d2 = p[2] - T[11];
  const double x = (T[0] * d0 + T[3] * d1) + T[6] * d2;
  const double y = (T[1] * d0 + T[4] * d1) + T[7] * d2;
  const double z = (T[2] * d0 + T[5] * d1) + T[8] * d2;
  double* r = resid + 3 * (size_t)a;
  if (!(z > 0.0)) {
    r[0] = r[1] = r[2] = __builtin_huge_val();
    return;
  }
  r[0] = (cx + fx * x / z) - obs_meas[3 * (size_t)a];
  r[1] = (cx + fx * (x - b) / z) - obs_meas[3 * (size_t)a + 1];
  r[2] = (cy + fy * y / z) - obs_meas[3 * (size_t)a + 2];
}

int check_image_args(const void* img, int n_img, int H, int W, int pitch) {
  VUS_REQUIRE(img != nullptr, "image pointer is null");
  VUS_REQUIRE(n_img >= 0 && n_img <= (1 << 20), "n_img=%d out of range [0, 2^20]", n_img);
  VUS_REQUIRE(H >= 7 && W >= 7, "image %dx%d too small (need >= 7x7)", W, H);
  VUS_REQUIRE(pitch >= W, "pitch %d < W %d", pitch, W);
  VUS_REQUIRE((long long)H * W <= (1ll << VUS_KEY_POS_BITS), "H*W=%lld exceeds 2^24", (long long)H * W);
  return VUS_OK;
}

struct TileGrid {
  unsigned blocks;
  int tiles_x, tiles_per_img;
};
TileGrid tile_grid(int n_img, int H, int W) {
  const int tx = (W + TW - 1) / TW, ty = (H + TH - 1) / TH;
  return TileGrid{(unsigned)(((n_img + 7) / 8) * 8 * tx * ty), tx, tx * ty};
}

typedef int v4i_t __attribute__((ext_vector_type(4)));
typedef int v8i_t __attribute__((ext_vector_type(8)));
typedef float v16f_t __attribute__((ext_vector_type(16)));
#ifndef VUS_HM_CHUNK
#define VUS_HM_CHUNK 128
#endif
constexpr int HM_CHUNK = VUS_HM_CHUNK;
constexpr int HM_KEY_SHIFT = HM_CHUNK == 256 ? 8 : HM_CHUNK == 128 ? 7 : HM_CHUNK == 64 ? 6 : -1;
static_assert(HM_KEY_SHIFT > 0, "HM_CHUNK must be 64, 128 or 256");
constexpr int HM_ROWB = 144;
constexpr int HM_SCALE_A = 0x7F7F7F7F;
constexpr int HM_SCALE_B = (int)(0x01010101u * (0x7F + HM_KEY_SHIFT));

#ifndef VUS_HM_QT
#define VUS_HM_QT 4
#endif
constexpr int HM_QT = VUS_HM_QT;
constexpr int HM_QWG = 4 * 32 * HM_QT;

__device__ __forceinline__ int spread_fp4(uint32_t b) {
  uint32_t x = (b | b << 12) & 0x000F000Fu;
  x = (x | x << 6) & 0x03030303u;
  return (int)(((x << 3 | x << 6) & 0x88888888u) | 0x22222222u);
}

__device__ __forceinline__ v4i_t spread_word(const uint32_t* lut, uint32_t w) {
  return v4i_t{(int)lut[w & 0xFFu], (int)lut[(w >> 8) & 0xFFu], (int)lut[(w >> 16) & 0xFFu], (int)lut[w >> 24]};
}

__device__ __forceinline__ v8i_t fp4_operand(v4i_t v) {
  return v8i_t{v[0], v[1], v[2], v[3], 0, 0, 0, 0};
}

__device__ __forceinline__ float max3f(float a, float b, float c) { return fmaxf(fmaxf(a, b), c); }

__device__ __forceinline__ float tile_best(const v16f_t& acc, float prev) {
  const float m0 = max3f(acc[0], acc[1], acc[2]), m1 = max3f(acc[3], acc[4], acc[5]), m2 = max3f(acc[6], acc[7], acc[8]),
              m3 = max3f(acc[9], acc[10], acc[11]), m4 = max3f(acc[12], acc[13], acc[14]),
              m5 = max3f(acc[15], prev + 32.0f, m0);
  return max3f(max3f(m1, m2, m3), m4, m5);
}

__global__ __launch_bounds__(256) __attribute__((amdgpu_waves_per_eu(3))) void hamming_match_mfma_kernel(
    const uint32_t* __restrict__ desc32, const int* __restrict__ kp_count, int max_kp, const int* __restrict__ q_index,
    const int* __restrict__ t_index, int max_dist, int32_t* __restrict__ idx_out, int32_t* __restrict__ dist_out) {
  __shared__ __attribute__((aligned(16))) uint8_t s_t[HM_CHUNK * HM_ROWB];
  __shared__ uint32_t s_lut[256];
  const int tid = threadIdx.x, lane = tid & 63, wave = tid >> 6;
  s_lut[tid] = spread_fp4(tid);
  __syncthreads();
  const int r = lane & 31, h = lane >> 5;
  const int p = blockIdx.y;
  const int qi = q_index[p], ti = t_index[p];
  const int nq = kp_count[qi];
  const int wq0 = blockIdx.x * HM_QWG + 32 * HM_QT * wave;
  const int q0 = wq0 + r;
  const int nt = blockIdx.x * HM_QWG < nq ? kp_count[ti] : 0;
  const bool wave_busy = wq0 < nq;
  v4i_t bq[HM_QT][4];
#pragma unroll
  for (int c = 0; c < HM_QT; ++c) {
    const int q = q0 + 32 * c;
    const uint32_t* dq = desc32 + ((size_t)qi * max_kp + min(q, max_kp - 1)) * 8 + h;
#pragma unroll
    for (int ks = 0; ks < 4; ++ks) bq[c][ks] = spread_word(s_lut, dq[2 * ks]);
  }
  v16f_t cinit;
#pragma unroll
  for (int reg = 0; reg < 16; ++reg) cinit[reg] = (float)(HM_CHUNK - 1 - ((reg & 3) + 8 * (reg >> 2)));
  int best[HM_QT];
#pragma unroll
  for (int c = 0; c < HM_QT; ++c) best[c] = INT_MIN;
  const uint32_t* dt = desc32 + (size_t)ti * max_kp * 8;
  constexpr int HM_ITEMS = HM_CHUNK * 8 / 256;
  uint32_t xw[HM_ITEMS];
#pragma unroll
  for (int u = 0; u < HM_ITEMS; ++u) xw[u] = nt > 0 ? dt[(size_t)min((tid + 256 * u) >> 3, nt - 1) * 8 + (tid & 7)] : 0u;
  for (int t0 = 0; t0 < nt; t0 += HM_CHUNK) {
    __syncthreads();
#pragma unroll
    for (int u = 0; u < HM_ITEMS; ++u) {
      const int item = tid + 256 * u;
      *reinterpret_cast<v4i_t*>(s_t + (item >> 3) * HM_ROWB + 16 * (item & 7)) = spread_word(s_lut, xw[u]);
    }
    __syncthreads();
    if (t0 + HM_CHUNK < nt) {
#pragma unroll
      for (int u = 0; u < HM_ITEMS; ++u)
        xw[u] = dt[(size_t)min(t0 + HM_CHUNK + ((tid + 256 * u) >> 3), nt - 1) * 8 + (tid & 7)];
    }
    if (!wave_busy) continue;
    const int ntile = min(HM_CHUNK, nt - t0 + 31) >> 5;
    float cb[HM_QT];
#pragma unroll
    for (int c = 0; c < HM_QT; ++c) cb[c] = -INFINITY;
    for (int tile = 0; tile < ntile; ++tile) {
      const uint8_t* arow = s_t + (32 * tile + r) * HM_ROWB + 16 * h;
      v16f_t acc[HM_QT];
#pragma unroll
      for (int ks = 0; ks < 4; ++ks) {
        const v8i_t a = fp4_operand(*reinterpret_cast<const v4i_t*>(arow + 32 * ks));
#pragma unroll
        for (int c = 0; c < HM_QT; ++c)
          acc[c] = __builtin_amdgcn_mfma_scale_f32_32x32x64_f8f6f4(a, fp4_operand(bq[c][ks]), ks == 0 ? cinit : acc[c],
                                                                   4, 4, 0, HM_SCALE_A, 0, HM_SCALE_B);
      }
      if (t0 + 32 * tile + 32 > nt) {
        const int tb = t0 + 32 * tile + 4 * h;
#pragma unroll
        for (int reg = 0; reg < 16; ++reg)
          if (tb + (reg & 3) + 8 * (reg >> 2) >= nt) {
#pragma unroll
            for (int c = 0; c < HM_QT; ++c) acc[c][reg] = -INFINITY;
          }
      }
#pragma unroll
      for (int c = 0; c < HM_QT; ++c) cb[c] = tile_best(acc[c], cb[c]);
    }
#pragma unroll
    for (int c = 0; c < HM_QT; ++c) {
      if (!(cb[c] > -INFINITY)) continue;
      const int k = (int)(cb[c] - 32.0f * (ntile - 1));
      const int train = t0 + 4 * h + (HM_CHUNK - 1 - (k & (HM_CHUNK - 1)));
      best[c] = max(best[c], (k >> HM_KEY_SHIFT) * 65536 + (0xFFFF - train));
    }
  }
#pragma unroll
  for (int c = 0; c < HM_QT; ++c) {
    const int b2 = max(best[c], __shfl_xor(best[c], 32));
    const int q = q0 + 32 * c;
    if (h == 0 && q < max_kp) {
      int bidx = -1, bd = 512;
      const int dot = b2 >> 16;
      if (q < nq && nt > 0 && dot >= -256) {
        bd = (256 - dot) >> 1;
        bidx = 0xFFFF - (b2 & 0xFFFF);
        if (bd > max_dist) bidx = -1;
      }
      idx_out[(size_t)p * max_kp + q] = bidx;
      dist_out[(size_t)p * max_kp + q] = bd;
    }
  }
}

__device__ __forceinline__ void resize_coeff(int d, int Ns, int Nd, int& i0, int& i1, int& w) {
  const int num = (2 * d + 1) * Ns - Nd, den = 2 * Nd;
  const int ix = num >= 0 ? (int)((unsigned)num / (unsigned)den) : -(int)((unsigned)(-num + den - 1) / (unsigned)den);
  const unsigned rem = (unsigned)(num - ix * den);
  w = (int)((rem * 2048u + (unsigned)Nd) / (unsigned)den);
  i0 = min(max(ix, 0), Ns - 1);
  i1 = min(max(ix + 1, 0), Ns - 1);
}

constexpr int RS_ROWS = 8;
__device__ __forceinline__ uint32_t window_byte(uint32_t w0, uint32_t w1, uint32_t w2, int o) {
  const uint32_t sel = o < 4 ? w0 : (o < 8 ? w1 : w2);
  return (sel >> (8 * (o & 3))) & 0xFFu;
}

constexpr int RS_THREADS = 64;
__global__ __launch_bounds__(RS_THREADS) void resize_bilinear_kernel(const uint8_t* __restrict__ src, int Hs, int Ws,
                                                              int pitch_s, uint8_t* __restrict__ dst, int Hd, int Wd,
                                                              int pitch_d) {
  __shared__ int s_y[RS_ROWS][3];
  const int xb = 4 * (blockIdx.x * RS_THREADS + threadIdx.x);
  const int ys = blockIdx.y * RS_ROWS;
  if (threadIdx.x < RS_ROWS) {
    int y0, y1, wy;
    resize_coeff(min(ys + (int)threadIdx.x, Hd - 1), Hs, Hd, y0, y1, wy);
    s_y[threadIdx.x][0] = y0 * pitch_s;
    s_y[threadIdx.x][1] = y1 * pitch_s;
    s_y[threadIdx.x][2] = wy;
  }
  __syncthreads();
  if (xb >= Wd) return;
  const uint8_t* s = src + (size_t)blockIdx.z * Hs * pitch_s;
  uint8_t* d = dst + (size_t)blockIdx.z * Hd * pitch_d;
  int x0[4], x1[4], wx[4];
#pragma unroll
  for (int j = 0; j < 4; ++j) resize_coeff(min(xb + j, Wd - 1), Ws, Wd, x0[j], x1[j], wx[j]);
  const int start = max(min(x0[0], Ws - 12), 0);
  const bool windowed = Ws >= 12 && x1[3] - start < 12;
  int o0[4], o1[4];
#pragma unroll
  for (int j = 0; j < 4; ++j) {
    o0[j] = x0[j] - start;
    o1[j] = x1[j] - start;
  }
  const int nx = min(4, Wd - xb);
#pragma unroll 2
  for (int r = 0; r < RS_ROWS; ++r) {
    const int y = ys + r;
    if (y >= Hd) break;
    const int r0 = s_y[r][0], r1 = s_y[r][1], wy = s_y[r][2];
    uint32_t out[4];
    if (windowed) {
      uint32_t t[3], b[3];
      __builtin_memcpy(t, s + r0 + start, 12);
      __builtin_memcpy(b, s + r1 + start, 12);
#pragma unroll
      for (int j = 0; j < 4; ++j) {
        const int top = (2048 - wx[j]) * (int)window_byte(t[0], t[1], t[2], o0[j]) + wx[j] * (int)window_byte(t[0], t[1], t[2], o1[j]);
        const int bot = (2048 - wx[j]) * (int)window_byte(b[0], b[1], b[2], o0[j]) + wx[j] * (int)window_byte(b[0], b[1], b[2], o1[j]);
        out[j] = (uint32_t)(((2048 - wy) * top + wy * bot + (1 << 21)) >> 22);
      }
    } else {
#pragma unroll
      for (int j = 0; j < 4; ++j) {
        const int top = (2048 - wx[j]) * s[r0 + x0[j]] + wx[j] * s[r0 + x1[j]];
        const int bot = (2048 - wx[j]) * s[r1 + x0[j]] + wx[j] * s[r1 + x1[j]];
        out[j] = (uint32_t)(((2048 - wy) * top + wy * bot + (1 << 21)) >> 22);
      }
    }
    uint8_t* o = d + (size_t)y * pitch_d + xb;
    if (nx == 4) {
      const uint32_t packed = out[0] | (out[1] << 8) | (out[2] << 16) | (out[3] << 24);
      __builtin_memcpy(o, &packed, 4);
    } else {
      for (int j = 0; j < nx; ++j) o[j] = (uint8_t)out[j];
    }
  }
}

__global__ __launch_bounds__(256) void pyramid_append_kernel(const uint32_t* __restrict__ lvl_keys,
                                                             const int* __restrict__ lvl_count,
                                                             const uint64_t* __restrict__ lvl_desc,
                                                             const uint8_t* __restrict__ lvl_angle, int lvl_max_kp,
                                                             int Hl, int Wl, int level, int H0, int W0, int max_kp,
                                                             uint32_t* __restrict__ kp_keys, int* __restrict__ kp_count,
                                                             uint64_t* __restrict__ desc, uint8_t* __restrict__ angle,
                                                             uint8_t* __restrict__ kp_level,
                                                             int32_t* __restrict__ kp_xy_q4) {
  const int n = blockIdx.x;
  const int base = kp_count[n];
  int cnt = min(lvl_count[n], lvl_max_kp);
  cnt = min(cnt, max_kp - base);
  __syncthreads();
  for (int t = threadIdx.x; t < cnt; t += 256) {
    const size_t li = (size_t)n * lvl_max_kp + t;
    const uint32_t key = lvl_keys[li];
    const int pos = (int)(key & VUS_KEY_POS_MASK), y = pos / Wl, x = pos - y * Wl;
    const int xq = (int)((((long long)(2 * x + 1) * 8 * W0 + Wl / 2) / Wl) - 8);
    const int yq = (int)((((long long)(2 * y + 1) * 8 * H0 + Hl / 2) / Hl) - 8);
    const int x0 = min(max((xq + 8) >> 4, 0), W0 - 1), y0 = min(max((yq + 8) >> 4, 0), H0 - 1);
    const size_t o = (size_t)n * max_kp + base + t;
    kp_keys[o] = (key & ~VUS_KEY_POS_MASK) | (uint32_t)(y0 * W0 + x0);
#pragma unroll
    for (int w = 0; w < 4; ++w) desc[4 * o + w] = lvl_desc[4 * li + w];
    angle[o] = lvl_angle[li];
    if (kp_level) kp_level[o] = (uint8_t)level;
    if (kp_xy_q4) {
      kp_xy_q4[2 * o] = xq;
      kp_xy_q4[2 * o + 1] = yq;
    }
  }
  if (threadIdx.x == 0) kp_count[n] = base + cnt;
}

__global__ void cross_check_kernel(const int32_t* __restrict__ idx_fwd, const int32_t* __restrict__ idx_bwd, int max_kp,
                                   long long total, int32_t* __restrict__ idx_out) {
  const long long t = (long long)blockIdx.x * blockDim.x + threadIdx.x;
  if (t >= total) return;
  const long long row = t / max_kp;
  const int i = (int)(t - row * max_kp);
  const int32_t j = idx_fwd[t];
  idx_out[t] = (j >= 0 && j < max_kp && idx_bwd[row * max_kp + j] == i) ? j : -1;
}

__global__ __launch_bounds__(SEL_THREADS) void select_grid_kernel(const uint32_t* __restrict__ cand_keys,
                                                                  const int* __restrict__ cand_count, int cand_cap,
                                                                  int H, int W, int grid_row, int grid_col, int per_cell,
                                                                  int max_kp, uint32_t* __restrict__ kp_keys,
                                                                  int* __restrict__ kp_count) {
  __shared__ uint32_t s_min[SEL_THREADS / 64];
  __shared__ uint32_t s_pick;
  const int tid = threadIdx.x, n = blockIdx.x;
  const uint32_t* keys = cand_keys + (size_t)n * cand_cap;
  const int cnt = min(cand_count[n], cand_cap);
  uint32_t* o = kp_keys + (size_t)n * max_kp;
  int out = 0;
  for (int cell = 0; cell < grid_row * grid_col && out < max_kp; ++cell) {
    const int cy = cell / grid_col, cx = cell - cy * grid_col;
    uint32_t last = 0;
    bool have_last = false;
    for (int j = 0; j < per_cell && out < max_kp; ++j) {
      uint32_t best = VUS_KEY_INVALID;
      for (int i = tid; i < cnt; i += SEL_THREADS) {
        const uint32_t k = keys[i];
        const int pos = (int)(k & VUS_KEY_POS_MASK), y = pos / W, x = pos - y * W;
        if (y * grid_row / H == cy && x * grid_col / W == cx && !(have_last && k <= last)) best = min(best, k);
      }
#pragma unroll
      for (int off = 32; off > 0; off >>= 1) best = min(best, (uint32_t)__shfl_xor((int)best, off));
      if ((tid & 63) == 0) s_min[tid >> 6] = best;
      __syncthreads();
      if (tid == 0) {
        uint32_t b = s_min[0];
        for (int w = 1; w < SEL_THREADS / 64; ++w) b = min(b, s_min[w]);
        s_pick = b;
      }
      __syncthreads();
      const uint32_t pick = s_pick;
      __syncthreads();
      if (pick == VUS_KEY_INVALID) break;
      if (tid == 0) o[out] = pick;
      ++out;
      last = pick;
      have_last = true;
    }
  }
  for (int i = out + tid; i < max_kp; i += SEL_THREADS) o[i] = VUS_KEY_INVALID;
  if (tid == 0) kp_count[n] = out;
}

}

extern "C" int vus_fast_score(const uint8_t* img, int n_img, int H, int W, int pitch, int thr,
                              uint8_t* score_out, void* stream) {
  if (int rc = check_image_args(img, n_img, H, W, pitch)) return rc;
  VUS_REQUIRE(score_out != nullptr, "score_out is null");
  VUS_REQUIRE(thr >= 1 && thr <= 254, "thr=%d out of range [1, 254]", thr);
  if (n_img == 0) return VUS_OK;
  const TileGrid g = tile_grid(n_img, H, W);
  fast_tile_kernel<true, false, false><<<g.blocks, NTHREADS, 0, vus::as_stream(stream)>>>(
      img, H, W, pitch, thr, nullptr, 0, score_out, nullptr, nullptr, 0, nullptr, n_img, g.tiles_x, g.tiles_per_img);
  VUS_CHECK_LAUNCH("fast_score");
  return VUS_OK;
}

extern "C" int vus_blur7(const uint8_t* img, int n_img, int H, int W, int pitch, uint8_t* out, void* stream) {
  if (int rc = check_image_args(img, n_img, H, W, pitch)) return rc;
  VUS_REQUIRE(out != nullptr, "out is null");
  if (n_img == 0) return VUS_OK;
  const TileGrid g = tile_grid(n_img, H, W);
  fast_tile_kernel<false, false, true><<<g.blocks, NTHREADS, 0, vus::as_stream(stream)>>>(
      img, H, W, pitch, 1, nullptr, 0, nullptr, out, nullptr, 0, nullptr, n_img, g.tiles_x, g.tiles_per_img);
  VUS_CHECK_LAUNCH("blur7");
  return VUS_OK;
}

extern "C" int vus_fast_detect(const uint8_t* img, int n_img, int H, int W, int pitch, int thr, int border,
                               uint8_t* blur_out, uint32_t* cand_keys, int cand_cap, int* cand_count,
                               void* stream) {
  if (int rc = check_image_args(img, n_img, H, W, pitch)) return rc;
  VUS_REQUIRE(cand_keys != nullptr && cand_count != nullptr, "candidate buffers are null");
  VUS_REQUIRE(cand_cap >= 1, "cand_cap=%d", cand_cap);
  VUS_REQUIRE(thr >= 1 && thr <= 254, "thr=%d out of range [1, 254]", thr);
  VUS_REQUIRE(border >= 0, "border=%d", border);
  if (n_img == 0) return VUS_OK;
  hipStream_t st = vus::as_stream(stream);
  const TileGrid g = tile_grid(n_img, H, W);
  if (blur_out)
    fast_tile_kernel<false, true, true><<<g.blocks, NTHREADS, 0, st>>>(
        img, H, W, pitch, thr, nullptr, border, nullptr, blur_out, cand_keys, cand_cap, cand_count, n_img, g.tiles_x,
        g.tiles_per_img);
  else
    fast_tile_kernel<false, true, false><<<g.blocks, NTHREADS, 0, st>>>(
        img, H, W, pitch, thr, nullptr, border, nullptr, nullptr, cand_keys, cand_cap, cand_count, n_img, g.tiles_x,
        g.tiles_per_img);
  VUS_CHECK_LAUNCH("fast_detect");
  return VUS_OK;
}

extern "C" int vus_fast_threshold_estimate(const uint8_t* img, int n_img, int H, int W, int pitch, int thr, int border,
                                           int max_kp, int sample_stride, int* hist, int* thr_img, void* stream) {
  if (int rc = check_image_args(img, n_img, H, W, pitch)) return rc;
  VUS_REQUIRE(hist != nullptr && thr_img != nullptr, "null buffer");
  VUS_REQUIRE(thr >= 1 && thr <= 254, "thr=%d out of range [1, 254]", thr);
  VUS_REQUIRE(border >= 0 && max_kp >= 1 && sample_stride >= 1, "border=%d max_kp=%d sample_stride=%d", border, max_kp, sample_stride);
  if (n_img == 0) return VUS_OK;
  hipStream_t st = vus::as_stream(stream);
  const TileGrid g = tile_grid(n_img, H, W);
  const int n_sampled = (g.tiles_per_img - sample_stride / 2 + sample_stride - 1) / sample_stride;
  VUS_CHECK_HIP(hipMemsetAsync(hist, 0, sizeof(int) * 256 * (size_t)n_img, st));
  const int floor = thr > VUS_FAST_SAMPLE_FLOOR ? thr : VUS_FAST_SAMPLE_FLOOR;
  if (n_sampled > 0)
    fast_sample_kernel<<<(unsigned)(((n_img + 7) / 8) * 8 * n_sampled), NTHREADS, 0, st>>>(
        img, H, W, pitch, floor, border, hist, n_img, g.tiles_x, g.tiles_per_img, sample_stride, n_sampled);
  fast_pick_threshold_kernel<<<(n_img + 3) / 4, 256, 0, st>>>(hist, n_img, thr, floor, max_kp, g.tiles_per_img,
                                                                 n_sampled > 0 ? n_sampled : 1, VUS_FAST_MARGIN_NUM,
                                                                 VUS_FAST_MARGIN_DEN, thr_img);
  VUS_CHECK_LAUNCH("fast_threshold_estimate");
  return VUS_OK;
}

extern "C" int vus_fast_detect_adaptive(const uint8_t* img, int n_img, int H, int W, int pitch, const int* thr_img, int border,
                                        uint8_t* blur_out, uint32_t* cand_keys, int cand_cap, int* cand_count, void* stream) {
  if (int rc = check_image_args(img, n_img, H, W, pitch)) return rc;
  VUS_REQUIRE(cand_keys != nullptr && cand_count != nullptr && thr_img != nullptr, "null buffer");
  VUS_REQUIRE(cand_cap >= 1 && border >= 0, "cand_cap=%d border=%d", cand_cap, border);
  if (n_img == 0) return VUS_OK;
  hipStream_t st = vus::as_stream(stream);
  const TileGrid g = tile_grid(n_img, H, W);
#ifndef VUS_FAST_LDS_PAD
#define VUS_FAST_LDS_PAD 0
#endif
  const bool regions = blur_out != nullptr && cand_cap >= 64 * VUS_CAND_REGIONS;
  if (regions) {
    cand_region_zero_kernel<<<(n_img * VUS_CAND_REGIONS + 255) / 256, 256, 0, st>>>(cand_keys, cand_cap, n_img);
    fast_tile_kernel<false, true, true, true><<<g.blocks, NTHREADS, VUS_FAST_LDS_PAD, st>>>(
        img, H, W, pitch, 0, thr_img, border, nullptr, blur_out, cand_keys, cand_cap, cand_count, n_img, g.tiles_x, g.tiles_per_img);
    cand_region_merge_kernel<<<n_img, 256, 0, st>>>(cand_keys, cand_cap, cand_count);
  } else if (blur_out)
    fast_tile_kernel<false, true, true><<<g.blocks, NTHREADS, VUS_FAST_LDS_PAD, st>>>(
        img, H, W, pitch, 0, thr_img, border, nullptr, blur_out, cand_keys, cand_cap, cand_count, n_img, g.tiles_x, g.tiles_per_img);
  else
    fast_tile_kernel<false, true, false><<<g.blocks, NTHREADS, 0, st>>>(
        img, H, W, pitch, 0, thr_img, border, nullptr, nullptr, cand_keys, cand_cap, cand_count, n_img, g.tiles_x, g.tiles_per_img);
  VUS_CHECK_LAUNCH("fast_detect_adaptive");
  return VUS_OK;
}

extern "C" int vus_fast_detect_retry(const uint8_t* img, int n_img, int H, int W, int pitch, int thr, const int* thr_img,
                                     int max_kp, int border, uint32_t* cand_keys, int cand_cap, int* cand_count,
                                     int* retry_list, int* retry_count, void* stream) {
  if (int rc = check_image_args(img, n_img, H, W, pitch)) return rc;
  VUS_REQUIRE(cand_keys && cand_count && thr_img && retry_list && retry_count, "null buffer");
  VUS_REQUIRE(thr >= 1 && thr <= 254 && max_kp >= 1 && cand_cap >= 1 && border >= 0, "thr=%d max_kp=%d cand_cap=%d border=%d", thr,
              max_kp, cand_cap, border);
  if (n_img == 0) return VUS_OK;
  hipStream_t st = vus::as_stream(stream);
  const TileGrid g = tile_grid(n_img, H, W);
  fast_retry_list_kernel<<<1, 1024, 0, st>>>(thr_img, thr, max_kp, n_img, cand_count, retry_list, retry_count);
  int n_cu = 256;
  {
    int dev = 0;
    if (hipGetDevice(&dev) != hipSuccess || hipDeviceGetAttribute(&n_cu, hipDeviceAttributeMultiprocessorCount, dev) != hipSuccess ||
        n_cu < 1)
      n_cu = 256;
  }
  fast_retry_kernel<<<8 * n_cu, NTHREADS, 0, st>>>(img, H, W, pitch, thr, border, cand_keys, cand_cap, cand_count, retry_list,
                                                   retry_count, g.tiles_x, g.tiles_per_img);
  VUS_CHECK_LAUNCH("fast_detect_retry");
  return VUS_OK;
}

extern "C" int vus_select_topk(const uint32_t* cand_keys, const int* cand_count, int n_img, int cand_cap,
                               int max_kp, uint32_t* kp_keys, int* kp_count, void* stream) {
  VUS_REQUIRE(cand_keys && cand_count && kp_keys && kp_count, "null buffer");
  VUS_REQUIRE(n_img >= 0, "n_img=%d", n_img);
  VUS_REQUIRE(cand_cap >= 1, "cand_cap=%d", cand_cap);
  VUS_REQUIRE(max_kp >= 1 && max_kp <= 8192, "max_kp=%d out of range [1, 8192]", max_kp);
  if (n_img == 0) return VUS_OK;
  int sort_n = 64;
  while (sort_n < max_kp) sort_n <<= 1;
  select_topk_kernel<<<n_img, SEL_THREADS, sort_n * sizeof(uint32_t), vus::as_stream(stream)>>>(
      cand_keys, cand_count, cand_cap, max_kp, sort_n, kp_keys, kp_count);
  VUS_CHECK_LAUNCH("select_topk");
  return VUS_OK;
}

static int orient_launch(const uint8_t* img, const uint8_t* blur, int n_img, int H, int W, int pitch, const uint32_t* kp_keys,
                         const int* kp_count, int max_kp, const int* order, uint64_t* desc_out, uint8_t* angle_out, void* stream) {
  if (int rc = check_image_args(img, n_img, H, W, pitch)) return rc;
  VUS_REQUIRE(blur && kp_keys && kp_count && desc_out && angle_out, "null buffer");
  VUS_REQUIRE(max_kp >= 1, "max_kp=%d", max_kp);
  if (n_img == 0) return VUS_OK;
  const int chunks = (max_kp + 4 * OR_KP_PER_WAVE - 1) / (4 * OR_KP_PER_WAVE);
  const long long blocks = (long long)((n_img + 7) / 8) * 8 * chunks;
  VUS_REQUIRE(blocks < (1ll << 31), "too many workgroups (%lld)", blocks);
  const bool aligned = ((reinterpret_cast<uintptr_t>(img) | reinterpret_cast<uintptr_t>(blur) | (uintptr_t)pitch |
                         (uintptr_t)W | ((uintptr_t)H * (uintptr_t)pitch)) & 3u) == 0;
#define VUS_OR_LAUNCH(EX, ORD)                                                                              \
  orient_rbrief_kernel<EX, ORD><<<(unsigned)blocks, 256, 0, vus::as_stream(stream)>>>(                      \
      img, blur, H, W, pitch, kp_keys, kp_count, max_kp, order, desc_out, angle_out, n_img, chunks)
  if (aligned && order) VUS_OR_LAUNCH(false, true);
  else if (aligned) VUS_OR_LAUNCH(false, false);
  else if (order) VUS_OR_LAUNCH(true, true);
  else VUS_OR_LAUNCH(true, false);
#undef VUS_OR_LAUNCH
  VUS_CHECK_LAUNCH("orient_rbrief");
  return VUS_OK;
}

extern "C" int vus_orient_rbrief(const uint8_t* img, const uint8_t* blur, int n_img, int H, int W, int pitch,
                                 const uint32_t* kp_keys, const int* kp_count, int max_kp,
                                 uint64_t* desc_out, uint8_t* angle_out, void* stream) {
  return orient_launch(img, blur, n_img, H, W, pitch, kp_keys, kp_count, max_kp, nullptr, desc_out, angle_out, stream);
}

extern "C" int vus_orient_order(const uint32_t* kp_keys, const int* kp_count, int n_img, int max_kp, int H, int W, int* order,
                                void* stream) {
  VUS_REQUIRE(kp_keys && kp_count && order, "null buffer");
  VUS_REQUIRE(n_img >= 0 && max_kp >= 1 && H >= 1 && W >= 1, "n_img=%d max_kp=%d H=%d W=%d", n_img, max_kp, H, W);
  if (n_img == 0) return VUS_OK;
  int cw = (W + OO_CELL - 1) / OO_CELL, ch = (H + OO_CELL - 1) / OO_CELL;
  VUS_REQUIRE((long long)cw * ch <= OO_MAX_CELLS, "image of %d x %d pixels has more than %d cells of %d x %d", W, H, OO_MAX_CELLS,
              OO_CELL, OO_CELL);
  orient_order_kernel<<<n_img, 256, 0, vus::as_stream(stream)>>>(kp_keys, kp_count, max_kp, W, cw, cw * ch, order);
  VUS_CHECK_LAUNCH("orient_order");
  return VUS_OK;
}

extern "C" int vus_orient_rbrief_ordered(const uint8_t* img, const uint8_t* blur, int n_img, int H, int W, int pitch,
                                         const uint32_t* kp_keys, const int* kp_count, int max_kp, const int* order,
                                         uint64_t* desc_out, uint8_t* angle_out, void* stream) {
  VUS_REQUIRE(order != nullptr, "null buffer");
  return orient_launch(img, blur, n_img, H, W, pitch, kp_keys, kp_count, max_kp, order, desc_out, angle_out, stream);
}

extern "C" int vus_hamming_match(const uint64_t* desc, const uint32_t* kp_keys, const int* kp_count,
                                 int max_kp, int H, int W, const int* q_index, const int* t_index, int n_pairs,
                                 int max_dy, int min_disp, int max_disp, int max_dist,
                                 int32_t* idx_out, int32_t* dist_out, void* stream) {
  VUS_REQUIRE(desc && kp_keys && kp_count && q_index && t_index && idx_out && dist_out, "null buffer");
  VUS_REQUIRE(max_kp >= 1 && W >= 1 && W < 65536 && H >= 1 && H < 65536, "max_kp=%d H=%d W=%d", max_kp, H, W);
  VUS_REQUIRE(n_pairs >= 0 && n_pairs <= 65535, "n_pairs=%d out of range [0, 65535]", n_pairs);
  if (n_pairs == 0) return VUS_OK;
  dim3 grid((max_kp + 255) / 256, n_pairs);
  const int h_rows = H;
  const size_t lds = sizeof(int) * ((size_t)2 * h_rows + 1 + 2 * (size_t)max_kp);
  if (max_dy >= 0 && h_rows <= 16384 && lds <= 96 * 1024) {
    if (lds > 48 * 1024)
      VUS_CHECK_HIP(hipFuncSetAttribute(reinterpret_cast<const void*>(hamming_match_rows_kernel),
                                        hipFuncAttributeMaxDynamicSharedMemorySize, (int)lds));
    hamming_match_rows_kernel<<<grid, 256, lds, vus::as_stream(stream)>>>(
        desc, kp_keys, kp_count, max_kp, W, h_rows, q_index, t_index, max_dy, min_disp, max_disp, max_dist, idx_out,
        dist_out);
  } else {
    if (max_dy >= 0)
      hamming_match_kernel<true><<<grid, 256, 0, vus::as_stream(stream)>>>(
          desc, kp_keys, kp_count, max_kp, W, q_index, t_index, max_dy, min_disp, max_disp, max_dist, idx_out, dist_out);
    else if (max_kp <= 65535)
      hamming_match_mfma_kernel<<<dim3((max_kp + HM_QWG - 1) / HM_QWG, n_pairs), 256, 0, vus::as_stream(stream)>>>(
          reinterpret_cast<const uint32_t*>(desc), kp_count, max_kp, q_index, t_index, max_dist, idx_out, dist_out);
    else
      hamming_match_kernel<false><<<grid, 256, 0, vus::as_stream(stream)>>>(
          desc, kp_keys, kp_count, max_kp, W, q_index, t_index, max_dy, min_disp, max_disp, max_dist, idx_out, dist_out);
  }
  VUS_CHECK_LAUNCH("hamming_match");
  return VUS_OK;
}

extern "C" int vus_track_ids(const int32_t* stereo_idx, const int32_t* track_idx, const uint32_t* kp_keys,
                             const int* kp_count, int n_frames, int max_kp, int H, int W, int64_t* ids_out,
                             double* feat_out, int64_t* n_ids_out, void* stream) {
  VUS_REQUIRE(stereo_idx && kp_keys && kp_count && ids_out && feat_out && n_ids_out, "null buffer");
  VUS_REQUIRE(n_frames >= 0 && max_kp >= 1 && max_kp <= 8192 && H >= 1 && W >= 1, "n_frames=%d max_kp=%d H=%d W=%d",
              n_frames, max_kp, H, W);
  VUS_REQUIRE(n_frames <= 1 || track_idx != nullptr, "track_idx is null");
  const size_t lds = (size_t)max_kp * (2 * sizeof(long long) + sizeof(int));
  if (lds > 48 * 1024)
    VUS_CHECK_HIP(hipFuncSetAttribute(reinterpret_cast<const void*>(track_ids_kernel),
                                      hipFuncAttributeMaxDynamicSharedMemorySize, (int)lds));
  track_ids_kernel<<<1, TRK_THREADS, lds, vus::as_stream(stream)>>>(
      stereo_idx, track_idx, kp_keys, kp_count, n_frames, max_kp, H, W, reinterpret_cast<long long*>(ids_out), feat_out,
      reinterpret_cast<long long*>(n_ids_out));
  VUS_CHECK_LAUNCH("track_ids");
  return VUS_OK;
}

extern "C" int vus_emit_stereo_factors(const int64_t* ids, const double* feat, const double* Rt, const double* cam,
                                       int n_frames, int max_kp, int first_frame, long long n_ids, int* frame_base,
                                       int* count, int* obs_frame, int64_t* obs_id, double* obs_meas, int64_t* lm_first,
                                       double* lm_point, void* stream) {
  VUS_REQUIRE(ids && feat && Rt && cam && frame_base && count && lm_first && lm_point, "null buffer");
  VUS_REQUIRE(obs_frame && obs_id && obs_meas, "null output buffer");
  VUS_REQUIRE(n_frames >= 0 && n_frames <= 65535 && max_kp >= 1 && first_frame >= 0 && n_ids >= 0,
              "n_frames=%d max_kp=%d first_frame=%d n_ids=%lld", n_frames, max_kp, first_frame, n_ids);
  VUS_REQUIRE((long long)n_frames * max_kp < (1ll << 31), "n_frames * max_kp overflows the int32 factor index");
  hipStream_t st = vus::as_stream(stream);
  if (n_ids > 0) VUS_CHECK_HIP(hipMemsetAsync(lm_first, 0xFF, sizeof(int64_t) * (size_t)n_ids, st));
  if (n_frames == 0) {
    VUS_CHECK_HIP(hipMemsetAsync(count, 0, sizeof(int), st));
    VUS_CHECK_HIP(hipMemsetAsync(frame_base, 0, sizeof(int), st));
    return VUS_OK;
  }
  emit_count_kernel<<<n_frames, EMIT_THREADS, 0, st>>>(reinterpret_cast<const long long*>(ids), max_kp, first_frame, n_ids,
                                                        frame_base, reinterpret_cast<unsigned long long*>(lm_first));
  emit_scan_kernel<<<1, 1024, 0, st>>>(frame_base, n_frames, count);
  emit_write_kernel<<<n_frames, EMIT_THREADS, 0, st>>>(reinterpret_cast<const long long*>(ids), feat, Rt, cam, max_kp,
                                                        first_frame, n_ids, frame_base, obs_frame,
                                                        reinterpret_cast<long long*>(obs_id), obs_meas,
                                                        reinterpret_cast<long long*>(lm_first), lm_point);
  VUS_CHECK_LAUNCH("emit_stereo_factors");
  return VUS_OK;
}

extern "C" int vus_stereo_initial_residuals(const double* Rt, const double* K, const double* lm_point,
                                            const int* obs_frame, const int64_t* obs_id, const double* obs_meas, int n,
                                            double* resid, void* stream) {
  VUS_REQUIRE(n >= 0, "n=%d", n);
  if (n == 0) return VUS_OK;
  VUS_REQUIRE(Rt && K && lm_point && obs_frame && obs_id && obs_meas && resid, "null buffer");
  stereo_initial_residuals_kernel<<<(n + 255) / 256, 256, 0, vus::as_stream(stream)>>>(
      Rt, K, lm_point, obs_frame, reinterpret_cast<const long long*>(obs_id), obs_meas, n, resid);
  VUS_CHECK_LAUNCH("stereo_initial_residuals");
  return VUS_OK;
}

extern "C" int vus_triangulate(const double* feat, int n, const double* cam, const double* Rt, double* out,
                               void* stream) {
  VUS_REQUIRE(feat && cam && Rt && out, "null buffer");
  VUS_REQUIRE(n >= 0, "n=%d", n);
  if (n == 0) return VUS_OK;
  triangulate_kernel<<<(n + 255) / 256, 256, 0, vus::as_stream(stream)>>>(feat, n, cam, Rt, out);
  VUS_CHECK_LAUNCH("triangulate");
  return VUS_OK;
}

extern "C" int vus_resize_bilinear(const uint8_t* src, int n_img, int Hs, int Ws, int pitch_s, uint8_t* dst, int Hd,
                                   int Wd, int pitch_d, void* stream) {
  if (int rc = check_image_args(src, n_img, Hs, Ws, pitch_s)) return rc;
  VUS_REQUIRE(dst != nullptr, "dst is null");
  VUS_REQUIRE(Hd >= 1 && Wd >= 1 && pitch_d >= Wd, "bad destination size %dx%d pitch %d", Hd, Wd, pitch_d);
  if (n_img == 0) return VUS_OK;
  VUS_REQUIRE(n_img <= 65535, "n_img=%d exceeds the grid's z extent", n_img);
  const dim3 grid((Wd + 4 * RS_THREADS - 1) / (4 * RS_THREADS), (Hd + RS_ROWS - 1) / RS_ROWS, n_img);
  resize_bilinear_kernel<<<grid, RS_THREADS, 0, vus::as_stream(stream)>>>(src, Hs, Ws, pitch_s, dst, Hd, Wd, pitch_d);
  VUS_CHECK_LAUNCH("resize_bilinear");
  return VUS_OK;
}

extern "C" int vus_pyramid_append(const uint32_t* lvl_keys, const int* lvl_count, const uint64_t* lvl_desc,
                                  const uint8_t* lvl_angle, int n_img, int lvl_max_kp, int Hl, int Wl, int level,
                                  int H0, int W0, int max_kp, uint32_t* kp_keys, int* kp_count, uint64_t* desc,
                                  uint8_t* angle, uint8_t* kp_level, int32_t* kp_xy_q4, void* stream) {
  VUS_REQUIRE(lvl_keys && lvl_count && lvl_desc && lvl_angle && kp_keys && kp_count && desc && angle, "null buffer");
  VUS_REQUIRE(n_img >= 0 && lvl_max_kp >= 1 && max_kp >= 1, "bad sizes: n_img=%d lvl_max_kp=%d max_kp=%d", n_img,
              lvl_max_kp, max_kp);
  VUS_REQUIRE(Hl >= 1 && Wl >= 1 && H0 >= 1 && W0 >= 1 && (long long)H0 * W0 <= (1ll << VUS_KEY_POS_BITS),
              "bad image sizes: level %dx%d, base %dx%d", Hl, Wl, H0, W0);
  VUS_REQUIRE(level >= 0 && level <= 255, "level=%d", level);
  if (n_img == 0) return VUS_OK;
  pyramid_append_kernel<<<n_img, 256, 0, vus::as_stream(stream)>>>(lvl_keys, lvl_count, lvl_desc, lvl_angle, lvl_max_kp,
                                                                   Hl, Wl, level, H0, W0, max_kp, kp_keys, kp_count,
                                                                   desc, angle, kp_level, kp_xy_q4);
  VUS_CHECK_LAUNCH("pyramid_append");
  return VUS_OK;
}

extern "C" int vus_cross_check(const int32_t* idx_fwd, const int32_t* idx_bwd, int n_pairs, int max_kp,
                               int32_t* idx_out, void* stream) {
  VUS_REQUIRE(idx_fwd && idx_bwd && idx_out, "null buffer");
  VUS_REQUIRE(n_pairs >= 0 && max_kp >= 1, "n_pairs=%d max_kp=%d", n_pairs, max_kp);
  const long long total = (long long)n_pairs * max_kp;
  if (total == 0) return VUS_OK;
  cross_check_kernel<<<(unsigned)((total + 255) / 256), 256, 0, vus::as_stream(stream)>>>(idx_fwd, idx_bwd, max_kp, total,
                                                                                       idx_out);
  VUS_CHECK_LAUNCH("cross_check");
  return VUS_OK;
}

extern "C" int vus_select_grid(const uint32_t* cand_keys, const int* cand_count, int n_img, int cand_cap, int H, int W,
                               int grid_row, int grid_col, int per_cell, int max_kp, uint32_t* kp_keys, int* kp_count,
                               void* stream) {
  VUS_REQUIRE(cand_keys && cand_count && kp_keys && kp_count, "null buffer");
  VUS_REQUIRE(n_img >= 0 && cand_cap >= 1 && max_kp >= 1, "n_img=%d cand_cap=%d max_kp=%d", n_img, cand_cap, max_kp);
  VUS_REQUIRE(H >= 1 && W >= 1 && H < 32768 && W < 32768, "H=%d W=%d", H, W);
  VUS_REQUIRE(grid_row >= 1 && grid_col >= 1 && grid_row <= 256 && grid_col <= 256 && per_cell >= 1,
              "grid %dx%d per_cell=%d", grid_row, grid_col, per_cell);
  if (n_img == 0) return VUS_OK;
  select_grid_kernel<<<n_img, SEL_THREADS, 0, vus::as_stream(stream)>>>(cand_keys, cand_count, cand_cap, H, W, grid_row,
                                                                        grid_col, per_cell, max_kp, kp_keys, kp_count);
  VUS_CHECK_LAUNCH("select_grid");
  return VUS_OK;
}
```

### visual-underwater-slam_amd/frontend.py

```python
from dataclasses import dataclass, field
from typing import List, Optional

import torch

from . import _lib


@dataclass
class ImageProcessorParams:
    fast_threshold: int = 10
    stereo_threshold: int = 5
    max_features: int = 2000
    border: int = 31
    min_disparity: int = 0
    max_disparity: int = 128
    stereo_max_distance: int = 64
    track_max_distance: int = 64
    cand_cap: int = 0
    grid_row: int = 0
    grid_col: int = 0
    grid_max_feature_num: int = 0
    cross_check: bool = False
    n_levels: int = 1
    scale_factor: float = 1.2
    adaptive_fast: bool = True
    fast_sample_stride: int = 32


def pyramid_layout(H: int, W: int, max_features: int, n_levels: int, scale_factor: float):
    sizes = [(int(round(H / scale_factor ** l)), int(round(W / scale_factor ** l))) for l in range(n_levels)]
    if n_levels == 1:
        return sizes, [max_features]
    f = 1.0 / scale_factor
    nd = max_features * (1.0 - f) / (1.0 - f ** n_levels)
    quotas, total = [], 0
    for _ in range(n_levels - 1):
        q = int(round(nd))
        quotas.append(q)
        total += q
        nd *= f
    quotas.append(max(max_features - total, 0))
    return sizes, quotas


@dataclass
class Feature:
    id: int
    u0: float
    v0: float
    u1: float
    v1: float


@dataclass
class CameraMeasurement:
    features: List[Feature] = field(default_factory=list)


class FrontendResult:

    def __init__(self, fe, n_frames):
        F = n_frames
        self.n_frames = F
        self.W = fe.W
        self.H = fe.H
        self.kp_keys = fe.kp_keys[:2 * F]
        self.kp_count = fe.kp_count[:2 * F]
        self.desc = fe.desc[:2 * F]
        self.angle = fe.angle[:2 * F]
        self.cand_count = fe.cand_count[:2 * F]
        self.stereo_idx = fe.match_idx[:F]
        self.stereo_dist = fe.match_dist[:F]
        self.kp_level = fe.kp_level[:2 * F] if fe.kp_level is not None else None
        self.kp_xy_q4 = fe.kp_xy_q4[:2 * F] if fe.kp_xy_q4 is not None else None
        self.track_idx = fe.match_idx[fe.max_frames:fe.max_frames + max(F - 1, 0)]
        self.track_dist = fe.match_dist[fe.max_frames:fe.max_frames + max(F - 1, 0)]

    def keypoints_xy_score(self):
        k = self.kp_keys.to(torch.int64) & 0xFFFFFFFF
        pos = k & 0xFFFFFF
        score = 255 - (k >> 24)
        valid = k != 0xFFFFFFFF
        y = torch.div(pos, self.W, rounding_mode="floor")
        x = pos - y * self.W
        score = torch.where(valid, score, torch.full_like(score, -1))
        return x.to(torch.int32), y.to(torch.int32), score.to(torch.int32)


class StereoOrbFrontend:

    def __init__(self, H: int, W: int, max_frames: int, params: Optional[ImageProcessorParams] = None,
                 device: str = "cuda:0"):
        _lib.require_gpu()
        _lib.load()
        self.p = params or ImageProcessorParams()
        if self.p.cand_cap <= 0:
            import dataclasses
            self.p = dataclasses.replace(self.p, cand_cap=max(32768, (int(H) * int(W)) // 16))
        self.stage_hook = None
        if self.p.grid_max_feature_num > 0:
            assert self.p.grid_row >= 1 and self.p.grid_col >= 1 and self.p.n_levels == 1, \
                "grid bucketing needs grid_row, grid_col >= 1 and a single pyramid level"
        self.H, self.W, self.max_frames = int(H), int(W), int(max_frames)
        self.device = torch.device(device)
        n_img, K, cap = 2 * self.max_frames, self.p.max_features, self.p.cand_cap
        dev = self.device
        self.blur = torch.empty((n_img, H, W), dtype=torch.uint8, device=dev)
        self.cand_keys = torch.empty((n_img, cap), dtype=torch.int32, device=dev)
        self.cand_count = torch.zeros((n_img,), dtype=torch.int32, device=dev)
        self.kp_keys = torch.empty((n_img, K), dtype=torch.int32, device=dev)
        self.kp_count = torch.zeros((n_img,), dtype=torch.int32, device=dev)
        self.desc = torch.empty((n_img, K, 4), dtype=torch.int64, device=dev)
        self.angle = torch.empty((n_img, K), dtype=torch.uint8, device=dev)
        self.kp_order = torch.empty((n_img, K), dtype=torch.int32, device=dev)
        self.match_idx = torch.empty((2 * self.max_frames, K), dtype=torch.int32, device=dev)
        self.match_dist = torch.empty((2 * self.max_frames, K), dtype=torch.int32, device=dev)
        f = torch.arange(self.max_frames, dtype=torch.int32, device=dev)
        self.stereo_q, self.stereo_t = (2 * f).contiguous(), (2 * f + 1).contiguous()
        self.track_q, self.track_t = (2 * f).contiguous(), (2 * f + 2).contiguous()
        self.kp_level = self.kp_xy_q4 = None
        self.levels = None
        self.cand_max_seen = torch.zeros((1,), dtype=torch.int32, device=dev)
        self.adaptive = bool(self.p.adaptive_fast and self.p.grid_max_feature_num <= 0)
        if self.adaptive:
            self.fast_hist = torch.zeros((n_img, 256), dtype=torch.int32, device=dev)
            self.fast_thr = torch.zeros((n_img,), dtype=torch.int32, device=dev)
            self.fast_retry_list = torch.zeros((n_img,), dtype=torch.int32, device=dev)
            self.fast_retry_count = torch.zeros((1,), dtype=torch.int32, device=dev)
        if self.p.cross_check:
            self.rev_idx = torch.empty((2 * self.max_frames, K), dtype=torch.int32, device=dev)
            self.rev_dist = torch.empty((2 * self.max_frames, K), dtype=torch.int32, device=dev)
        if self.p.n_levels > 1:
            sizes, quotas = pyramid_layout(H, W, K, self.p.n_levels, self.p.scale_factor)
            assert all(h >= 2 * self.p.border + 8 and w >= 2 * self.p.border + 8 for h, w in sizes), \
                "pyramid level smaller than the detector border"
            self.kp_level = torch.zeros((n_img, K), dtype=torch.uint8, device=dev)
            self.kp_xy_q4 = torch.zeros((n_img, K, 2), dtype=torch.int32, device=dev)
            self.levels = []
            for l, ((h, w), q) in enumerate(zip(sizes, quotas)):
                q = max(q, 1)
                self.levels.append(dict(
                    H=h, W=w, quota=q,
                    img=None if l == 0 else torch.empty((n_img, h, w), dtype=torch.uint8, device=dev),
                    blur=self.blur if l == 0 else torch.empty((n_img, h, w), dtype=torch.uint8, device=dev),
                    keys=torch.empty((n_img, q), dtype=torch.int32, device=dev),
                    count=torch.zeros((n_img,), dtype=torch.int32, device=dev),
                    desc=torch.empty((n_img, q, 4), dtype=torch.int64, device=dev),
                    angle=torch.empty((n_img, q), dtype=torch.uint8, device=dev)))

    def process(self, images: torch.Tensor, check: bool = True) -> FrontendResult:
        assert images.dtype == torch.uint8 and images.is_cuda and images.is_contiguous()
        F = images.shape[0]
        assert images.shape[1:] == (2, self.H, self.W) and 1 <= F <= self.max_frames
        p, H, W, K = self.p, self.H, self.W, self.p.max_features
        n_img = 2 * F
        st = _lib.current_stream_ptr()
        ptr = _lib.ptr
        mark = self.stage_hook or (lambda name: None)
        mark("begin")
        if self.levels is None:
            self.cand_count[:n_img].zero_()
            if self.adaptive:
                _lib.call("vus_fast_threshold_estimate", ptr(images), n_img, H, W, W, p.fast_threshold, p.border, K,
                          p.fast_sample_stride, ptr(self.fast_hist), ptr(self.fast_thr), st)
                mark("fast_threshold")
                _lib.call("vus_fast_detect_adaptive", ptr(images), n_img, H, W, W, ptr(self.fast_thr), p.border,
                          ptr(self.blur), ptr(self.cand_keys), p.cand_cap, ptr(self.cand_count), st)
                _lib.call("vus_fast_detect_retry", ptr(images), n_img, H, W, W, p.fast_threshold, ptr(self.fast_thr), K,
                          p.border, ptr(self.cand_keys), p.cand_cap, ptr(self.cand_count), ptr(self.fast_retry_list),
                          ptr(self.fast_retry_count), st)
            else:
                _lib.call("vus_fast_detect", ptr(images), n_img, H, W, W, p.fast_threshold, p.border,
                          ptr(self.blur), ptr(self.cand_keys), p.cand_cap, ptr(self.cand_count), st)
            mark("fast_detect")
            if p.grid_max_feature_num > 0:
                _lib.call("vus_select_grid", ptr(self.cand_keys), ptr(self.cand_count), n_img, p.cand_cap, H, W,
                          p.grid_row, p.grid_col, p.grid_max_feature_num, K, ptr(self.kp_keys), ptr(self.kp_count), st)
            else:
                _lib.call("vus_select_topk", ptr(self.cand_keys), ptr(self.cand_count), n_img, p.cand_cap, K,
                          ptr(self.kp_keys), ptr(self.kp_count), st)
            mark("select_topk")
            self._orient(ptr(images), ptr(self.blur), n_img, H, W, ptr(self.kp_keys), ptr(self.kp_count), K, ptr(self.desc),
                         ptr(self.angle), st)
            mark("orient_rbrief")
        else:
            self._process_pyramid(images, n_img, st)
            mark("pyramid_detect_describe")
        _lib.call("vus_hamming_match", ptr(self.desc), ptr(self.kp_keys), ptr(self.kp_count), K, H, W,
                  ptr(self.stereo_q), ptr(self.stereo_t), F, p.stereo_threshold, p.min_disparity,
                  p.max_disparity, p.stereo_max_distance, ptr(self.match_idx), ptr(self.match_dist), st)
        mark("hamming_stereo")
        if F > 1:
            _lib.call("vus_hamming_match", ptr(self.desc), ptr(self.kp_keys), ptr(self.kp_count), K, H, W,
                      ptr(self.track_q), ptr(self.track_t), F - 1, -1, 0, 0, p.track_max_distance,
                      ptr(self.match_idx[self.max_frames:]), ptr(self.match_dist[self.max_frames:]), st)
        mark("hamming_track")
        if p.cross_check:
            _lib.call("vus_hamming_match", ptr(self.desc), ptr(self.kp_keys), ptr(self.kp_count), K, H, W,
                      ptr(self.stereo_t), ptr(self.stereo_q), F, p.stereo_threshold, -p.max_disparity,
                      -p.min_disparity, p.stereo_max_distance, ptr(self.rev_idx), ptr(self.rev_dist), st)
            _lib.call("vus_cross_check", ptr(self.match_idx), ptr(self.rev_idx), F, K, ptr(self.match_idx), st)
            if F > 1:
                _lib.call("vus_hamming_match", ptr(self.desc), ptr(self.kp_keys), ptr(self.kp_count), K, H, W,
                          ptr(self.track_t), ptr(self.track_q), F - 1, -1, 0, 0, p.track_max_distance,
                          ptr(self.rev_idx[self.max_frames:]), ptr(self.rev_dist[self.max_frames:]), st)
                _lib.call("vus_cross_check", ptr(self.match_idx[self.max_frames:]), ptr(self.rev_idx[self.max_frames:]),
                          F - 1, K, ptr(self.match_idx[self.max_frames:]), st)
            mark("cross_check")
        if self.levels is None:
            torch.maximum(self.cand_max_seen, self.cand_count[:n_img].max().reshape(1), out=self.cand_max_seen)
        mark("end")
        if check:
            self.check_overflow(n_img)
        return FrontendResult(self, F)

    def _process_pyramid(self, images, n_img, st):
        p, K, ptr = self.p, self.p.max_features, _lib.ptr
        self.kp_count[:n_img].zero_()
        self.kp_keys[:n_img].fill_(-1)
        self.pyr_cand_max = torch.zeros((1,), dtype=torch.int32, device=self.device)
        prev = images
        for l, L in enumerate(self.levels):
            h, w = L["H"], L["W"]
            if l > 0:
                P = self.levels[l - 1]
                _lib.call("vus_resize_bilinear", ptr(prev), n_img, P["H"], P["W"], P["W"], ptr(L["img"]), h, w, w, st)
                prev = L["img"]
            self.cand_count[:n_img].zero_()
            if self.adaptive:
                _lib.call("vus_fast_threshold_estimate", ptr(prev), n_img, h, w, w, p.fast_threshold, p.border, L["quota"],
                          p.fast_sample_stride, ptr(self.fast_hist), ptr(self.fast_thr), st)
                _lib.call("vus_fast_detect_adaptive", ptr(prev), n_img, h, w, w, ptr(self.fast_thr), p.border, ptr(L["blur"]),
                          ptr(self.cand_keys), p.cand_cap, ptr(self.cand_count), st)
                _lib.call("vus_fast_detect_retry", ptr(prev), n_img, h, w, w, p.fast_threshold, ptr(self.fast_thr), L["quota"],
                          p.border, ptr(self.cand_keys), p.cand_cap, ptr(self.cand_count), ptr(self.fast_retry_list),
                          ptr(self.fast_retry_count), st)
            else:
                _lib.call("vus_fast_detect", ptr(prev), n_img, h, w, w, p.fast_threshold, p.border, ptr(L["blur"]),
                          ptr(self.cand_keys), p.cand_cap, ptr(self.cand_count), st)
            torch.maximum(self.pyr_cand_max, self.cand_count[:n_img].max().reshape(1), out=self.pyr_cand_max)
            _lib.call("vus_select_topk", ptr(self.cand_keys), ptr(self.cand_count), n_img, p.cand_cap, L["quota"],
                      ptr(L["keys"]), ptr(L["count"]), st)
            self._orient(ptr(prev), ptr(L["blur"]), n_img, h, w, ptr(L["keys"]), ptr(L["count"]), L["quota"], ptr(L["desc"]),
                         ptr(L["angle"]), st)
            _lib.call("vus_pyramid_append", ptr(L["keys"]), ptr(L["count"]), ptr(L["desc"]), ptr(L["angle"]), n_img,
                      L["quota"], h, w, l, self.H, self.W, K, ptr(self.kp_keys), ptr(self.kp_count), ptr(self.desc),
                      ptr(self.angle), ptr(self.kp_level), ptr(self.kp_xy_q4), st)

    def _orient(self, img_p, blur_p, n_img, h, w, keys_p, count_p, k, desc_p, angle_p, st):
        if ((h + 63) // 64) * ((w + 63) // 64) <= 1024:
            _lib.call("vus_orient_order", keys_p, count_p, n_img, k, h, w, _lib.ptr(self.kp_order), st)
            _lib.call("vus_orient_rbrief_ordered", img_p, blur_p, n_img, h, w, w, keys_p, count_p, k, _lib.ptr(self.kp_order),
                      desc_p, angle_p, st)
        else:
            _lib.call("vus_orient_rbrief", img_p, blur_p, n_img, h, w, w, keys_p, count_p, k, desc_p, angle_p, st)

    def check_overflow(self, n_img=None):
        if self.levels is not None:
            worst = int(self.pyr_cand_max.item())
            if worst > self.p.cand_cap:
                raise _lib.VusError(f"FAST produced {worst} candidates in one pyramid level, more than cand_cap="
                                    f"{self.p.cand_cap}: raise ImageProcessorParams.cand_cap")
            return
        worst = int(self.cand_max_seen.item())
        self.cand_max_seen.zero_()
        if worst > self.p.cand_cap:
            raise _lib.VusError(f"FAST produced {worst} candidates in one image, more than cand_cap="
                                f"{self.p.cand_cap}: raise ImageProcessorParams.cand_cap")

    def feature_tracks(self, res: FrontendResult):
        F, K = res.n_frames, self.p.max_features
        dev = self.device
        ids = torch.empty((F, K), dtype=torch.int64, device=dev)
        feats = torch.empty((F, K, 4), dtype=torch.float64, device=dev)
        n_ids = torch.zeros((1,), dtype=torch.int64, device=dev)
        ptr = _lib.ptr
        _lib.call("vus_track_ids", ptr(res.stereo_idx), ptr(res.track_idx) if F > 1 else None, ptr(res.kp_keys),
                  ptr(res.kp_count), F, K, self.H, self.W, ptr(ids), ptr(feats), ptr(n_ids),
                  _lib.current_stream_ptr())
        return ids, feats, int(n_ids.item())

    def stereo_factors(self, ids: torch.Tensor, feats: torch.Tensor, n_ids: int, Rt: torch.Tensor, cam: torch.Tensor,
                       first_frame: int = 1):
        F, K = ids.shape
        dev = ids.device
        assert Rt.shape == (F, 12) and Rt.dtype == torch.float64 and Rt.is_contiguous() and cam.numel() == 8
        cap = F * K
        base = torch.empty((F + 1,), dtype=torch.int32, device=dev)
        count = torch.zeros((1,), dtype=torch.int32, device=dev)
        of = torch.empty((cap,), dtype=torch.int32, device=dev)
        oi = torch.empty((cap,), dtype=torch.int64, device=dev)
        om = torch.empty((cap, 3), dtype=torch.float64, device=dev)
        first = torch.empty((max(n_ids, 1),), dtype=torch.int64, device=dev)
        pt = torch.zeros((max(n_ids, 1), 3), dtype=torch.float64, device=dev)
        ptr = _lib.ptr
        _lib.call("vus_emit_stereo_factors", ptr(ids), ptr(feats), ptr(Rt), ptr(cam), F, K, int(first_frame), int(n_ids),
                  ptr(base), ptr(count), ptr(of), ptr(oi), ptr(om), ptr(first), ptr(pt), _lib.current_stream_ptr())
        n = int(count.item())
        return {"obs_frame": of[:n], "obs_id": oi[:n], "obs_meas": om[:n], "lm_first": first[:n_ids],
                "lm_point": pt[:n_ids]}

    def camera_measurements(self, res: FrontendResult) -> List[CameraMeasurement]:
        ids, feats, _ = self.feature_tracks(res)
        ids, feats = ids.cpu().numpy(), feats.cpu().numpy()
        out = []
        for f in range(res.n_frames):
            msg = CameraMeasurement()
            for i in (ids[f] >= 0).nonzero()[0].tolist():
                u0, v0, u1, v1 = feats[f, i]
                msg.features.append(Feature(id=int(ids[f, i]), u0=float(u0), v0=float(v0), u1=float(u1), v1=float(v1)))
            out.append(msg)
        return out


def triangulate(feat: torch.Tensor, cam: torch.Tensor, Rt: torch.Tensor) -> torch.Tensor:
    _lib.require_gpu()
    assert feat.dtype == torch.float64 and feat.is_cuda and feat.is_contiguous() and feat.shape[1] == 4
    out = torch.empty((feat.shape[0], 6), dtype=torch.float64, device=feat.device)
    _lib.call("vus_triangulate", _lib.ptr(feat), feat.shape[0], _lib.ptr(cam), _lib.ptr(Rt), _lib.ptr(out),
              _lib.current_stream_ptr())
    return out
```

Measured before the change: 178,000.

## Store blur and raw image planes in 16x8 block-tiled layout for orientation/BRIEF

```diff
diff --git a/include/vus_tiled.h b/include/vus_tiled.h
--- /dev/null
+++ b/include/vus_tiled.h
@@ -0,0 +1,35 @@
+#ifndef VUS_TILED_H
+#define VUS_TILED_H
+#include "vus.h"
+
+#define VUS_TILE_BW 16
+#define VUS_TILE_BH 8
+
+#if defined(__HIPCC__)
+#define VUS_TILED_QUAL __host__ __device__ static inline
+#else
+#define VUS_TILED_QUAL static inline
+#endif
+
+VUS_TILED_QUAL unsigned vus_tiled_offset(int y, int x, int W) {
+  const unsigned uy = (unsigned)y, ux = (unsigned)x;
+  return (uy / VUS_TILE_BH) * ((unsigned)W * VUS_TILE_BH) + (ux / VUS_TILE_BW) * (VUS_TILE_BW * VUS_TILE_BH) +
+         (uy % VUS_TILE_BH) * VUS_TILE_BW + ux % VUS_TILE_BW;
+}
+
+#ifdef __cplusplus
+extern "C" {
+#endif
+
+int vus_fast_detect_adaptive_tiled(const uint8_t* img, int n_img, int H, int W, int pitch, const int* thr_img, int border,
+                                   uint8_t* blur_tiled, uint8_t* img_tiled, uint32_t* cand_keys, int cand_cap,
+                                   int* cand_count, void* stream);
+
+int vus_orient_rbrief_tiled(const uint8_t* img_tiled, const uint8_t* blur_tiled, int n_img, int H, int W,
+                            const uint32_t* kp_keys, const int* kp_count, int max_kp, const int* order,
+                            uint64_t* desc_out, uint8_t* angle_out, void* stream);
+
+#ifdef __cplusplus
+}
+#endif
+#endif
diff --git a/visual-underwater-slam_amd/_lib.py b/visual-underwater-slam_amd/_lib.py
--- a/visual-underwater-slam_amd/_lib.py
+++ b/visual-underwater-slam_amd/_lib.py
@@ -62,6 +62,8 @@
     "vus_ba_point_check": [_P, c_int, _P, _P],
     "vus_ba_point_covariance": [_P, _P, _P, _P, _P, c_int, _P, _P],
     "vus_nav_border_covariance": [c_int, c_int, _P, _P, _P, _P, _P, _P, _P, _P],
+    "vus_fast_detect_adaptive_tiled": [_P, c_int, c_int, c_int, c_int, _P, c_int, _P, _P, _P, c_int, _P, _P],
+    "vus_orient_rbrief_tiled": [_P, _P, c_int, c_int, c_int, _P, _P, c_int, _P, _P, _P, _P],
     "vus_between_check": [_P, c_int, _P],
     "vus_between_linearize": [_P, _P, _P, _P, _P, _P],
     "vus_between_assemble": [_P, _P, c_int, _P, _P, _P],
diff --git a/visual-underwater-slam_amd/csrc/frontend.hip b/visual-underwater-slam_amd/csrc/frontend.hip
--- a/visual-underwater-slam_amd/csrc/frontend.hip
+++ b/visual-underwater-slam_amd/csrc/frontend.hip
@@ -1,6 +1,8 @@
 #include "vus_common.h"
+#include <type_traits>
 #define VUS_TABLE_QUAL __device__ constexpr
 #include "../../include/vus_orb_tables.h"
+#include "../../include/vus_tiled.h"
 
 namespace {
 
@@ -176,6 +178,7 @@
 __device__ __attribute__((aligned(16))) const BlurMfmaTable g_blur_mfma_table = make_blur_mfma_table();
 typedef int v4i32_t __attribute__((ext_vector_type(4)));
 
+template <bool TILED = false>
 __device__ __forceinline__ void blur_tile_mfma(const uint32_t* s_img, uint8_t* __restrict__ blur_out, int n, int H, int W,
                                                int x0, int y0, int tid, int j_first, int j_step) {
   static_assert(IMG_ROWS == 32 && TW % 16 == 0 && (IMG_DW * 4) % 8 == 0, "blur_tile_mfma: K = the 32 staged rows");
@@ -221,7 +224,9 @@
 #ifdef VUS_BLUR_EXP_NOSTORE
       if (v != 0x12345678u) continue;
 #endif
-      if (ly < TH && gy < H) {
+      if (TILED) {
+        if (ly < TH && gy < H && gx < W) __builtin_memcpy(blur_out + (size_t)n * H * W + vus_tiled_offset(gy, gx, W), &v, 4);
+      } else if (ly < TH && gy < H) {
         uint8_t* o = blur_out + ((size_t)n * H + gy) * W + gx;
         if (gx + 3 < W) {
           __builtin_memcpy(o, &v, 4);
@@ -243,12 +248,12 @@
   return 0;
 }
 #endif
-template <bool WRITE_SCORE, bool DETECT, bool BLUR, bool HIST = false, bool REGIONS = false>
+template <bool WRITE_SCORE, bool DETECT, bool BLUR, bool HIST = false, bool REGIONS = false, bool TILED = false>
 __device__ __forceinline__ void fast_tile_body(
     const uint8_t* __restrict__ img, int H, int W, int pitch, int thr, int border,
     uint8_t* __restrict__ score_out, uint8_t* __restrict__ blur_out,
     uint32_t* __restrict__ cand_keys, int cand_cap, int* __restrict__ cand_count, int* __restrict__ hist,
-    int n, int tile, int tiles_x) {
+    int n, int tile, int tiles_x, uint8_t* __restrict__ raw_out = nullptr) {
   __shared__ __attribute__((aligned(8))) uint32_t s_img[IMG_ROWS * IMG_DW];
   __shared__ uint32_t s_score[(WRITE_SCORE || DETECT) ? SC_ROWS * SC_DW : 1];
   constexpr bool STRIP = VUS_FAST_STRIP && (WRITE_SCORE || DETECT);
@@ -266,6 +271,7 @@
   static_assert(IMG_ROWS * IMG_DW >= TW * TH / 4, "candidate list must fit in the image tile");
   static_assert(!LATE_BLUR || AUX_DW >= TW * TH / 4, "candidate list must fit in the strip tables' buffer");
   uint32_t* const s_keys = LATE_BLUR ? s_h : s_img;
+  static_assert(!TILED || LATE_BLUR, "the block-tiled planes are written by the late-smoothing detection launch");
 
   const int tid = threadIdx.x;
   const int x0 = (tile % tiles_x) * TW, y0 = (tile / tiles_x) * TH;
@@ -598,8 +604,24 @@
       uint32_t* const list = cand_keys + (size_t)n * cand_cap + (REGIONS ? (size_t)(tile & (VUS_CAND_REGIONS - 1)) * rcap : 0);
       int* const counter = REGIONS ? reinterpret_cast<int*>(list) : &cand_count[n];
       if (LATE_BLUR) {
-        if (tid == NTHREADS - 64 && cnt > 0) s_base = atomicAdd(counter, cnt);
-        if (tid < NTHREADS - 64) blur_tile_mfma(s_img, blur_out, n, H, W, x0, y0, tid, tid >> 6, NTHREADS / 64 - 1);
+        const bool leader = tid == NTHREADS - 64 && cnt > 0;
+        int base = 0;
+        if (leader) base = atomicAdd(counter, cnt);
+        if (TILED && tid >= NTHREADS - 64) {
+          const uint8_t* s8 = reinterpret_cast<const uint8_t*>(s_img);
+          uint8_t* const ro = raw_out + (size_t)n * H * W;
+          for (int i = tid - (NTHREADS - 64); i < TH * (TW / 16); i += 64) {
+            const int ly = i / (TW / 16), cb = i - ly * (TW / 16);
+            const int gy = y0 + ly, gx = x0 + 16 * cb;
+            if (gy < H && gx < W) {
+              const uint8_t* sp = s8 + (ly + 4) * (4 * IMG_DW) + 8 + 16 * cb;
+              const uint2 a = *reinterpret_cast<const uint2*>(sp), b = *reinterpret_cast<const uint2*>(sp + 8);
+              *reinterpret_cast<uint4*>(ro + vus_tiled_offset(gy, gx, W)) = make_uint4(a.x, a.y, b.x, b.y);
+            }
+          }
+        }
+        if (leader) s_base = base;
+        if (tid < NTHREADS - 64) blur_tile_mfma<TILED>(s_img, blur_out, n, H, W, x0, y0, tid, tid >> 6, NTHREADS / 64 - 1);
       } else {
         if (tid == 0 && cnt > 0) s_base = atomicAdd(counter, cnt);
       }
@@ -625,6 +647,19 @@
   const int tile = slot - (slot / tiles_per_img) * tiles_per_img;
   fast_tile_body<WRITE_SCORE, DETECT, BLUR, false, REGIONS>(img, H, W, pitch, thr_img ? thr_img[n] : thr, border, score_out, blur_out,
                                                             cand_keys, cand_cap, cand_count, nullptr, n, tile, tiles_x);
+}
+
+template <bool REGIONS>
+__global__ __launch_bounds__(NTHREADS, VUS_FAST_WPE) void fast_tile_tiled_kernel(
+    const uint8_t* __restrict__ img, int H, int W, int pitch, const int* __restrict__ thr_img, int border,
+    uint8_t* __restrict__ blur_out, uint8_t* __restrict__ raw_out, uint32_t* __restrict__ cand_keys, int cand_cap,
+    int* __restrict__ cand_count, int n_img, int tiles_x, int tiles_per_img) {
+  const int xcd = blockIdx.x & 7, slot = blockIdx.x >> 3;
+  const int n = (slot / tiles_per_img) * 8 + xcd;
+  if (n >= n_img) return;
+  const int tile = slot - (slot / tiles_per_img) * tiles_per_img;
+  fast_tile_body<false, true, true, false, REGIONS, true>(img, H, W, pitch, thr_img[n], border, nullptr, blur_out, cand_keys,
+                                                          cand_cap, cand_count, nullptr, n, tile, tiles_x, raw_out);
 }
 
 __global__ void cand_region_zero_kernel(uint32_t* __restrict__ cand_keys, int cand_cap, int n_img) {
@@ -889,6 +924,63 @@
   }
 };
 
+template <int RADIUS, int DW>
+struct TiledPatchRegs {
+  static_assert(DW % 2 == 0, "row width must be a multiple of the vector width");
+  typedef typename PatchVec<2>::type vec_t;
+  static constexpr int ROWS = 2 * RADIUS + 1;
+  static constexpr int HW = DW / 2;
+  static constexpr int N = ROWS * HW;
+  static constexpr int ITERS = (N + 63) / 64;
+  vec_t v[ITERS];
+  uint32_t row[ITERS];
+  uint32_t off0[ITERS], off8[ITERS];
+
+  __device__ __forceinline__ void init(int lane) {
+#pragma unroll
+    for (int u = 0; u < ITERS; ++u) {
+      const int t = min(lane + 64 * u, N - 1);
+      const uint32_t r = (uint32_t)(t / HW), q0 = 8u * (uint32_t)(t % HW), q8 = q0 + 8u;
+      row[u] = r;
+      off0[u] = 16u * r + 128u * (q0 >> 4) + (q0 & 8u);
+      off8[u] = 16u * r + 128u * (q8 >> 4) + (q8 & 8u);
+    }
+  }
+  __device__ __forceinline__ void load(const uint8_t* __restrict__ src, int H, int W, int y, int x, int lane) {
+    const int xa = (x - RADIUS) & ~7, y0 = y - RADIUS;
+    const bool inside = y0 >= 0 && y + RADIUS < H && xa >= 0 && xa + 4 * DW <= W;
+    if (inside) {
+      const uint8_t* base = src + vus_tiled_offset(y0 & ~7, xa & ~15, W) + 16 * (y0 & 7);
+      const uint32_t ys = (uint32_t)(y0 & 7), ystep = 8u * (uint32_t)W - 128u;
+      const bool x8 = (xa & 8) != 0;
+#pragma unroll
+      for (int u = 0; u < ITERS; ++u) {
+        const uint32_t off = ((ys + row[u]) >> 3) * ystep + (x8 ? off8[u] : off0[u]);
+        v[u] = *reinterpret_cast<const vec_t*>(base + (size_t)off);
+      }
+    } else {
+#pragma unroll
+      for (int u = 0; u < ITERS; ++u) {
+        const int t = min(lane + 64 * u, N - 1);
+        const int r = t / HW, c = t - r * HW;
+        const int gy = clampi(y0 + r, 0, H - 1), gx = xa + 8 * c;
+#pragma unroll
+        for (int k = 0; k < 2; ++k) {
+          uint32_t w = 0;
+#pragma unroll
+          for (int b = 0; b < 4; ++b) w |= (uint32_t)src[vus_tiled_offset(gy, clampi(gx + 4 * k + b, 0, W - 1), W)] << (8 * b);
+          v[u][k] = w;
+        }
+      }
+    }
+  }
+  __device__ __forceinline__ void store(uint32_t* __restrict__ dst, int lane) const {
+#pragma unroll
+    for (int u = 0; u < ITERS; ++u)
+      if (lane + 64 * u < N) *reinterpret_cast<uint2*>(dst + 2 * (lane + 64 * u)) = make_uint2(v[u][0], v[u][1]);
+  }
+};
+
 __device__ __forceinline__ int fold32(int x, int y) {
   auto r = __builtin_amdgcn_permlane32_swap((uint32_t)x, (uint32_t)y, false, false);
   return (int)(r[0] + r[1]);
@@ -932,17 +1024,17 @@
 struct RotOffTable {
   uint32_t v[VUS_N_ANGLE_BINS * 64 * 4];
 };
-constexpr RotOffTable make_rot_off_table() {
+constexpr RotOffTable make_rot_off_table(int row_bytes) {
   RotOffTable r{};
   for (int e = 0; e < VUS_N_ANGLE_BINS * 256; ++e) {
     const int bin = e / 256, test = e - 256 * bin, w = test >> 6, lane = test & 63;
-    const int oa = VUS_RBRIEF_ROT[4 * e + 1] * (4 * BR_DW) + VUS_RBRIEF_ROT[4 * e];
-    const int ob = VUS_RBRIEF_ROT[4 * e + 3] * (4 * BR_DW) + VUS_RBRIEF_ROT[4 * e + 2];
+    const int oa = VUS_RBRIEF_ROT[4 * e + 1] * row_bytes + VUS_RBRIEF_ROT[4 * e];
+    const int ob = VUS_RBRIEF_ROT[4 * e + 3] * row_bytes + VUS_RBRIEF_ROT[4 * e + 2];
     r.v[(bin * 64 + lane) * 4 + w] = ((uint32_t)oa & 0xFFFFu) | ((uint32_t)ob << 16);
   }
   return r;
 }
-__device__ __attribute__((aligned(16))) const RotOffTable g_rot_off_table = make_rot_off_table();
+__device__ __attribute__((aligned(16))) const RotOffTable g_rot_off_table = make_rot_off_table(4 * BR_DW);
 
 #ifndef VUS_OR_WPE
 #define VUS_OR_WPE 4
@@ -955,13 +1047,29 @@
 constexpr int OR_NV = OR_ROWS * (OR_DW / OR_VW);
 constexpr int OR_WT = 192;
 
+template <bool TILED> struct OrGeom {
+  static constexpr int ALIGN = 4, OR_DW = ::OR_DW, BR_DW = ::BR_DW;
+  typedef PatchRegs<OR_R, OR_DW, OR_VW, false> Disc;
+  typedef PatchRegs<BR_R, BR_DW, OR_VW, false> Brief;
+};
+template <> struct OrGeom<true> {
+  static constexpr int ALIGN = 8, OR_DW = 10, BR_DW = 12;
+  typedef TiledPatchRegs<OR_R, OR_DW> Disc;
+  typedef TiledPatchRegs<BR_R, BR_DW> Brief;
+};
+static_assert(OrGeom<true>::OR_DW == OR_DW && 2 * OR_R + 1 + 7 <= 4 * OrGeom<true>::OR_DW && 2 * BR_R + 1 + 7 <= 4 * OrGeom<true>::BR_DW,
+              "tiled patch rows: 8-byte aligned starts, same centroid vectors");
+__device__ __attribute__((aligned(16))) const RotOffTable g_rot_off_table_tiled = make_rot_off_table(4 * OrGeom<true>::BR_DW);
+
+template <int ALIGN>
 struct DiscWeightTable {
-  uint32_t v[4 * OR_WT * 4];
+  uint32_t v[ALIGN * OR_WT * 4];
 };
-constexpr DiscWeightTable make_disc_weight_table() {
+template <int ALIGN>
+constexpr DiscWeightTable<ALIGN> make_disc_weight_table() {
   constexpr int umax[16] = {15, 15, 15, 15, 14, 14, 14, 13, 13, 12, 11, 10, 9, 8, 6, 3};
-  DiscWeightTable r{};
-  for (int e = 0; e < 4 * OR_WT; ++e) {
+  DiscWeightTable<ALIGN> r{};
+  for (int e = 0; e < ALIGN * OR_WT; ++e) {
     const int sh = e / OR_WT, t = e - sh * OR_WT;
     if (t >= OR_NV) continue;
     const int row = t / (OR_DW / 2), c = t - row * (OR_DW / 2);
@@ -977,7 +1085,8 @@
   }
   return r;
 }
-__device__ __attribute__((aligned(16))) const DiscWeightTable g_disc_weight_table = make_disc_weight_table();
+__device__ __attribute__((aligned(16))) const DiscWeightTable<4> g_disc_weight_table = make_disc_weight_table<4>();
+__device__ __attribute__((aligned(16))) const DiscWeightTable<8> g_disc_weight_table8 = make_disc_weight_table<8>();
 
 constexpr int OO_CELL = 64, OO_MAX_CELLS = 1024;
 __global__ __launch_bounds__(256) void orient_order_kernel(const uint32_t* __restrict__ kp_keys, const int* __restrict__ kp_count,
@@ -1027,13 +1136,15 @@
   for (int j = cnt + tid; j < max_kp; j += 256) ord[j] = j;
 }
 
-template <bool EXACT, bool ORDERED>
+template <bool EXACT, bool ORDERED, bool TILED = false>
 __global__ __launch_bounds__(256) __attribute__((amdgpu_waves_per_eu(VUS_OR_WPE, 8))) void orient_rbrief_kernel(
     const uint8_t* __restrict__ img, const uint8_t* __restrict__ blur, int H, int W, int pitch,
     const uint32_t* __restrict__ kp_keys, const int* __restrict__ kp_count, int max_kp, const int* __restrict__ order,
     uint64_t* __restrict__ desc_out, uint8_t* __restrict__ angle_out, int n_img, int chunks_per_img) {
-  __shared__ uint4 s_w[4 * OR_WT];
-  __shared__ __attribute__((aligned(8))) uint32_t s_blur[4][2][BR_ROWS * BR_DW];
+  typedef OrGeom<TILED> G;
+  static_assert(!(TILED && EXACT), "tiled planes are always read from aligned starts");
+  __shared__ uint4 s_w[G::ALIGN * OR_WT];
+  __shared__ __attribute__((aligned(8))) uint32_t s_blur[4][2][BR_ROWS * G::BR_DW];
   const int lane = threadIdx.x & 63;
   const int wave = __builtin_amdgcn_readfirstlane(threadIdx.x >> 6);
   const int xcd = blockIdx.x & 7, slot = blockIdx.x >> 3;
@@ -1041,9 +1152,9 @@
   const int chunk = slot - (slot / chunks_per_img) * chunks_per_img;
   if (n >= n_img) return;
   {
-    const uint4* wt = reinterpret_cast<const uint4*>(g_disc_weight_table.v);
-#pragma unroll
-    for (int i = 0; i < 4 * OR_WT / 256; ++i) s_w[threadIdx.x + 256 * i] = wt[threadIdx.x + 256 * i];
+    const uint4* wt = reinterpret_cast<const uint4*>(TILED ? g_disc_weight_table8.v : g_disc_weight_table.v);
+#pragma unroll
+    for (int i = 0; i < G::ALIGN * OR_WT / 256; ++i) s_w[threadIdx.x + 256 * i] = wt[threadIdx.x + 256 * i];
   }
   const uint8_t* im = img + (size_t)n * H * pitch;
   const uint8_t* bl = blur + (size_t)n * H * W;
@@ -1064,11 +1175,17 @@
     bin_cos[q] = VUS_ANGLE_COS[bq];
     bin_sin[q] = VUS_ANGLE_SIN[bq];
   }
-  PatchRegs<OR_R, OR_DW, OR_VW, EXACT> pr[OR_GRP];
-  PatchRegs<BR_R, BR_DW, OR_VW, EXACT> pb;
-#pragma unroll
-  for (int kk = 0; kk < OR_GRP; ++kk) pr[kk].init(pitch, lane);
-  pb.init(W, lane);
+  typename std::conditional<TILED, typename G::Disc, PatchRegs<OR_R, OR_DW, OR_VW, EXACT>>::type pr[OR_GRP];
+  typename std::conditional<TILED, typename G::Brief, PatchRegs<BR_R, BR_DW, OR_VW, EXACT>>::type pb;
+  if constexpr (TILED) {
+#pragma unroll
+    for (int kk = 0; kk < OR_GRP; ++kk) pr[kk].init(lane);
+    pb.init(lane);
+  } else {
+#pragma unroll
+    for (int kk = 0; kk < OR_GRP; ++kk) pr[kk].init(pitch, lane);
+    pb.init(W, lane);
+  }
   int mom_dy[3];
 #pragma unroll
   for (int u = 0; u < 3; ++u) mom_dy[u] = min(lane + 64 * u, OR_NV - 1) / (OR_DW / 2) - OR_R;
@@ -1086,21 +1203,25 @@
     for (int kk = 0; kk < OR_GRP; ++kk) {
       const int k = OR_GRP * g + kk;
 #ifndef VUS_OR_EXP_NORAW
-      if (k < n_live)
-        pr[kk].load(im, H, W, pitch, __builtin_amdgcn_readlane(my_y, k), __builtin_amdgcn_readlane(my_x, k), lane);
+      if (k < n_live) {
+        if constexpr (TILED) pr[kk].load(im, H, W, __builtin_amdgcn_readlane(my_y, k), __builtin_amdgcn_readlane(my_x, k), lane);
+        else pr[kk].load(im, H, W, pitch, __builtin_amdgcn_readlane(my_y, k), __builtin_amdgcn_readlane(my_x, k), lane);
+      }
 #else
       for (int u = 0; u < 3; ++u) pr[kk].v[u] = typename PatchVec<OR_VW>::type{(uint32_t)lane, (uint32_t)k};
 #endif
     }
-    if (g == 8 / OR_GRP - 1)
-      pb.load(bl, H, W, W, __builtin_amdgcn_readlane(my_y, 0), __builtin_amdgcn_readlane(my_x, 0), lane);
+    if (g == 8 / OR_GRP - 1) {
+      if constexpr (TILED) pb.load(bl, H, W, __builtin_amdgcn_readlane(my_y, 0), __builtin_amdgcn_readlane(my_x, 0), lane);
+      else pb.load(bl, H, W, W, __builtin_amdgcn_readlane(my_y, 0), __builtin_amdgcn_readlane(my_x, 0), lane);
+    }
 #pragma unroll
     for (int kk = 0; kk < OR_GRP; ++kk) {
       const int k = OR_GRP * g + kk;
       pa[k] = 0;
       pq[k] = 0;
       if (k < n_live) {
-        const int sh = EXACT ? 0 : (__builtin_amdgcn_readlane(my_x, k) - OR_R) & 3;
+        const int sh = EXACT ? 0 : (__builtin_amdgcn_readlane(my_x, k) - OR_R) & (G::ALIGN - 1);
         const uint4* wt = s_w + sh * OR_WT + lane;
         uint32_t sx = 0;
         int si = 0, sy = 0;
@@ -1153,7 +1274,7 @@
   }
 
   uint32_t wlo = 0, whi = 0;
-  const uint4* rot = reinterpret_cast<const uint4*>(g_rot_off_table.v) + lane;
+  const uint4* rot = reinterpret_cast<const uint4*>(TILED ? g_rot_off_table_tiled.v : g_rot_off_table.v) + lane;
   uint4 to = rot[__builtin_amdgcn_readlane(my_bin, 0) * 64];
   for (int k = 0; k < n_live; ++k) {
     uint32_t* patch = s_blur[wave][k & 1];
@@ -1162,13 +1283,14 @@
     const int cx = __builtin_amdgcn_readlane(my_x, k);
     if (k + 1 < n_live) {
 #ifndef VUS_OR_EXP_NOBLUR
-      pb.load(bl, H, W, W, __builtin_amdgcn_readlane(my_y, k + 1), __builtin_amdgcn_readlane(my_x, k + 1), lane);
+      if constexpr (TILED) pb.load(bl, H, W, __builtin_amdgcn_readlane(my_y, k + 1), __builtin_amdgcn_readlane(my_x, k + 1), lane);
+      else pb.load(bl, H, W, W, __builtin_amdgcn_readlane(my_y, k + 1), __builtin_amdgcn_readlane(my_x, k + 1), lane);
 #endif
       to = rot[__builtin_amdgcn_readlane(my_bin, 8 * (k + 1)) * 64];
     }
     __builtin_amdgcn_fence(__ATOMIC_ACQ_REL, "wavefront");
-    const int sh_blur = EXACT ? 0 : (cx - BR_R) & 3;
-    const uint8_t* c = reinterpret_cast<const uint8_t*>(patch) + BR_R * (4 * BR_DW) + BR_R + sh_blur;
+    const int sh_blur = EXACT ? 0 : (cx - BR_R) & (G::ALIGN - 1);
+    const uint8_t* c = reinterpret_cast<const uint8_t*>(patch) + BR_R * (4 * G::BR_DW) + BR_R + sh_blur;
     const uint32_t tw[4] = {cto.x, cto.y, cto.z, cto.w};
 #pragma unroll
     for (int w = 0; w < 4; ++w) {
@@ -2005,6 +2127,38 @@
   return VUS_OK;
 }
 
+static int check_tiled_args(const void* a, const void* b, int H, int W) {
+  VUS_REQUIRE(a != nullptr && b != nullptr, "tiled plane pointer is null");
+  VUS_REQUIRE(W % VUS_TILE_BW == 0 && H % VUS_TILE_BH == 0, "tiled planes need W %% %d == 0 and H %% %d == 0 (got %dx%d)",
+              VUS_TILE_BW, VUS_TILE_BH, W, H);
+  VUS_REQUIRE(((reinterpret_cast<uintptr_t>(a) | reinterpret_cast<uintptr_t>(b)) & 15u) == 0, "tiled planes must be 16-byte aligned");
+  return VUS_OK;
+}
+
+extern "C" int vus_fast_detect_adaptive_tiled(const uint8_t* img, int n_img, int H, int W, int pitch, const int* thr_img,
+                                              int border, uint8_t* blur_tiled, uint8_t* img_tiled, uint32_t* cand_keys,
+                                              int cand_cap, int* cand_count, void* stream) {
+  if (int rc = check_image_args(img, n_img, H, W, pitch)) return rc;
+  if (int rc = check_tiled_args(blur_tiled, img_tiled, H, W)) return rc;
+  VUS_REQUIRE(cand_keys != nullptr && cand_count != nullptr && thr_img != nullptr, "null buffer");
+  VUS_REQUIRE(cand_cap >= 1 && border >= 0, "cand_cap=%d border=%d", cand_cap, border);
+  if (n_img == 0) return VUS_OK;
+  hipStream_t st = vus::as_stream(stream);
+  const TileGrid g = tile_grid(n_img, H, W);
+  static_assert(TW % VUS_TILE_BW == 0 && TH % VUS_TILE_BH == 0, "a detector tile is whole blocks");
+  if (cand_cap >= 64 * VUS_CAND_REGIONS) {
+    cand_region_zero_kernel<<<(n_img * VUS_CAND_REGIONS + 255) / 256, 256, 0, st>>>(cand_keys, cand_cap, n_img);
+    fast_tile_tiled_kernel<true><<<g.blocks, NTHREADS, 0, st>>>(img, H, W, pitch, thr_img, border, blur_tiled, img_tiled,
+                                                                cand_keys, cand_cap, cand_count, n_img, g.tiles_x, g.tiles_per_img);
+    cand_region_merge_kernel<<<n_img, 256, 0, st>>>(cand_keys, cand_cap, cand_count);
+  } else {
+    fast_tile_tiled_kernel<false><<<g.blocks, NTHREADS, 0, st>>>(img, H, W, pitch, thr_img, border, blur_tiled, img_tiled,
+                                                                 cand_keys, cand_cap, cand_count, n_img, g.tiles_x, g.tiles_per_img);
+  }
+  VUS_CHECK_LAUNCH("fast_detect_adaptive_tiled");
+  return VUS_OK;
+}
+
 extern "C" int vus_fast_detect_retry(const uint8_t* img, int n_img, int H, int W, int pitch, int thr, const int* thr_img,
                                      int max_kp, int border, uint32_t* cand_keys, int cand_cap, int* cand_count,
                                      int* retry_list, int* retry_count, void* stream) {
@@ -2091,6 +2245,27 @@
                                          uint64_t* desc_out, uint8_t* angle_out, void* stream) {
   VUS_REQUIRE(order != nullptr, "null buffer");
   return orient_launch(img, blur, n_img, H, W, pitch, kp_keys, kp_count, max_kp, order, desc_out, angle_out, stream);
+}
+
+extern "C" int vus_orient_rbrief_tiled(const uint8_t* img_tiled, const uint8_t* blur_tiled, int n_img, int H, int W,
+                                       const uint32_t* kp_keys, const int* kp_count, int max_kp, const int* order,
+                                       uint64_t* desc_out, uint8_t* angle_out, void* stream) {
+  if (int rc = check_image_args(img_tiled, n_img, H, W, W)) return rc;
+  if (int rc = check_tiled_args(img_tiled, blur_tiled, H, W)) return rc;
+  VUS_REQUIRE(kp_keys && kp_count && desc_out && angle_out, "null buffer");
+  VUS_REQUIRE(max_kp >= 1, "max_kp=%d", max_kp);
+  if (n_img == 0) return VUS_OK;
+  const int chunks = (max_kp + 4 * OR_KP_PER_WAVE - 1) / (4 * OR_KP_PER_WAVE);
+  const long long blocks = (long long)((n_img + 7) / 8) * 8 * chunks;
+  VUS_REQUIRE(blocks < (1ll << 31), "too many workgroups (%lld)", blocks);
+  if (order)
+    orient_rbrief_kernel<false, true, true><<<(unsigned)blocks, 256, 0, vus::as_stream(stream)>>>(
+        img_tiled, blur_tiled, H, W, W, kp_keys, kp_count, max_kp, order, desc_out, angle_out, n_img, chunks);
+  else
+    orient_rbrief_kernel<false, false, true><<<(unsigned)blocks, 256, 0, vus::as_stream(stream)>>>(
+        img_tiled, blur_tiled, H, W, W, kp_keys, kp_count, max_kp, order, desc_out, angle_out, n_img, chunks);
+  VUS_CHECK_LAUNCH("orient_rbrief_tiled");
+  return VUS_OK;
 }
 
 extern "C" int vus_hamming_match(const uint64_t* desc, const uint32_t* kp_keys, const int* kp_count,
diff --git a/visual-underwater-slam_amd/frontend.py b/visual-underwater-slam_amd/frontend.py
--- a/visual-underwater-slam_amd/frontend.py
+++ b/visual-underwater-slam_amd/frontend.py
@@ -4,6 +4,25 @@
 import torch
 
 from . import _lib
+
+
+TILE_BW, TILE_BH = 16, 8
+
+
+def tiled_supported(H: int, W: int) -> bool:
+    return H % TILE_BH == 0 and W % TILE_BW == 0
+
+
+def tile_planes(planes: torch.Tensor) -> torch.Tensor:
+    n, H, W = planes.shape
+    return (planes.reshape(n, H // TILE_BH, TILE_BH, W // TILE_BW, TILE_BW).permute(0, 1, 3, 2, 4)
+            .reshape(n, H * W).contiguous())
+
+
+def untile_planes(tiled: torch.Tensor, H: int, W: int) -> torch.Tensor:
+    n = tiled.shape[0]
+    return (tiled.reshape(n, H // TILE_BH, W // TILE_BW, TILE_BH, TILE_BW).permute(0, 1, 3, 2, 4)
+            .reshape(n, H, W).contiguous())
 
 
 @dataclass
@@ -105,7 +124,14 @@
         self.device = torch.device(device)
         n_img, K, cap = 2 * self.max_frames, self.p.max_features, self.p.cand_cap
         dev = self.device
-        self.blur = torch.empty((n_img, H, W), dtype=torch.uint8, device=dev)
+        self.tiled = bool(self.p.n_levels == 1 and self.p.adaptive_fast and self.p.grid_max_feature_num <= 0
+                          and tiled_supported(self.H, self.W))
+        if self.tiled:
+            self.blur_tiled = torch.empty((n_img, H * W), dtype=torch.uint8, device=dev)
+            self.img_tiled = torch.empty((n_img, H * W), dtype=torch.uint8, device=dev)
+            self._blur = None
+        else:
+            self._blur = torch.empty((n_img, H, W), dtype=torch.uint8, device=dev)
         self.cand_keys = torch.empty((n_img, cap), dtype=torch.int32, device=dev)
         self.cand_count = torch.zeros((n_img,), dtype=torch.int32, device=dev)
         self.kp_keys = torch.empty((n_img, K), dtype=torch.int32, device=dev)
@@ -142,7 +168,7 @@
                 self.levels.append(dict(
                     H=h, W=w, quota=q,
                     img=None if l == 0 else torch.empty((n_img, h, w), dtype=torch.uint8, device=dev),
-                    blur=self.blur if l == 0 else torch.empty((n_img, h, w), dtype=torch.uint8, device=dev),
+                    blur=self._blur if l == 0 else torch.empty((n_img, h, w), dtype=torch.uint8, device=dev),
                     keys=torch.empty((n_img, q), dtype=torch.int32, device=dev),
                     count=torch.zeros((n_img,), dtype=torch.int32, device=dev),
                     desc=torch.empty((n_img, q, 4), dtype=torch.int64, device=dev),
@@ -164,14 +190,19 @@
                 _lib.call("vus_fast_threshold_estimate", ptr(images), n_img, H, W, W, p.fast_threshold, p.border, K,
                           p.fast_sample_stride, ptr(self.fast_hist), ptr(self.fast_thr), st)
                 mark("fast_threshold")
-                _lib.call("vus_fast_detect_adaptive", ptr(images), n_img, H, W, W, ptr(self.fast_thr), p.border,
-                          ptr(self.blur), ptr(self.cand_keys), p.cand_cap, ptr(self.cand_count), st)
+                if self.tiled:
+                    _lib.call("vus_fast_detect_adaptive_tiled", ptr(images), n_img, H, W, W, ptr(self.fast_thr), p.border,
+                              ptr(self.blur_tiled), ptr(self.img_tiled), ptr(self.cand_keys), p.cand_cap,
+                              ptr(self.cand_count), st)
+                else:
+                    _lib.call("vus_fast_detect_adaptive", ptr(images), n_img, H, W, W, ptr(self.fast_thr), p.border,
+                              ptr(self._blur), ptr(self.cand_keys), p.cand_cap, ptr(self.cand_count), st)
                 _lib.call("vus_fast_detect_retry", ptr(images), n_img, H, W, W, p.fast_threshold, ptr(self.fast_thr), K,
                           p.border, ptr(self.cand_keys), p.cand_cap, ptr(self.cand_count), ptr(self.fast_retry_list),
                           ptr(self.fast_retry_count), st)
             else:
                 _lib.call("vus_fast_detect", ptr(images), n_img, H, W, W, p.fast_threshold, p.border,
-                          ptr(self.blur), ptr(self.cand_keys), p.cand_cap, ptr(self.cand_count), st)
+                          ptr(self._blur), ptr(self.cand_keys), p.cand_cap, ptr(self.cand_count), st)
             mark("fast_detect")
             if p.grid_max_feature_num > 0:
                 _lib.call("vus_select_grid", ptr(self.cand_keys), ptr(self.cand_count), n_img, p.cand_cap, H, W,
@@ -180,8 +211,11 @@
                 _lib.call("vus_select_topk", ptr(self.cand_keys), ptr(self.cand_count), n_img, p.cand_cap, K,
                           ptr(self.kp_keys), ptr(self.kp_count), st)
             mark("select_topk")
-            self._orient(ptr(images), ptr(self.blur), n_img, H, W, ptr(self.kp_keys), ptr(self.kp_count), K, ptr(self.desc),
-                         ptr(self.angle), st)
+            if self.tiled:
+                self._orient_tiled(n_img, st)
+            else:
+                self._orient(ptr(images), ptr(self._blur), n_img, H, W, ptr(self.kp_keys), ptr(self.kp_count), K,
+                             ptr(self.desc), ptr(self.angle), st)
             mark("orient_rbrief")
         else:
             self._process_pyramid(images, n_img, st)
@@ -255,6 +289,21 @@
         else:
             _lib.call("vus_orient_rbrief", img_p, blur_p, n_img, h, w, w, keys_p, count_p, k, desc_p, angle_p, st)
 
+    def _orient_tiled(self, n_img, st):
+        H, W, K, ptr = self.H, self.W, self.p.max_features, _lib.ptr
+        order = None
+        if ((H + 63) // 64) * ((W + 63) // 64) <= 1024:
+            _lib.call("vus_orient_order", ptr(self.kp_keys), ptr(self.kp_count), n_img, K, H, W, ptr(self.kp_order), st)
+            order = ptr(self.kp_order)
+        _lib.call("vus_orient_rbrief_tiled", ptr(self.img_tiled), ptr(self.blur_tiled), n_img, H, W, ptr(self.kp_keys),
+                  ptr(self.kp_count), K, order, ptr(self.desc), ptr(self.angle), st)
+
+    @property
+    def blur(self) -> torch.Tensor:
+        if self.tiled:
+            return untile_planes(self.blur_tiled, self.H, self.W)
+        return self._blur
+
     def check_overflow(self, n_img=None):
         if self.levels is not None:
             worst = int(self.pyr_cand_max.item())
```

New measurement: 184,200 (median of 6 runs). 1.04x the previous value.
